# smdesai/mlx-swift-audio

Measured on AMD Instinct MI355X. Metric: audio-sec/s (Whisper large-v3-turbo b=32) at 1/2/4/8 GPU; codec samples/s, higher is better.
Workload: dtype bf16; 1 GPU; Whisper large-v3-turbo bf16, batch=32x30 s synthetic clips per MI355X, log-mel+encode+greedy decode (T=0, timestamps, max_tokens 448, one window per clip), random-init N(0,0.02^2) weights; clips_per_gpu=32, global_batch=32, parallelism=dp1, replicas=3, exchange=none, schedule=pipelined

## Files before the change

include/mia.h:

```cpp
#ifndef MIA_H
#define MIA_H

#include <stddef.h>
#include <stdint.h>

#ifdef __cplusplus
extern "C" {
#endif

typedef struct mia_ctx mia_ctx;
typedef struct mia_whisper mia_whisper;
typedef struct mia_codec mia_codec;
typedef struct mia_lm mia_lm;
typedef struct mia_s3tok mia_s3tok;

typedef enum {
  MIA_OK = 0,
  MIA_ERR_INVALID_ARGUMENT = -1,
  MIA_ERR_MODEL_NOT_LOADED = -2,
  MIA_ERR_INVALID_AUDIO = -3,
  MIA_ERR_OUT_OF_MEMORY = -4,
  MIA_ERR_DEVICE = -5,
  MIA_ERR_UNSUPPORTED = -6
} mia_status;
// ... 32 lines not shown

int mia_dp_shard_range(int n_items, int rank, int world, int* lo, int* hi);
int mia_dp_shard_cap(int n_items, int world);
int mia_dp_unpack_host(const int32_t* gathered, int n_items, int world, int L, int32_t* dense);
int mia_dp_available(void);
int mia_dp_unique_id(mia_ctx* ctx, void* id128);
int mia_dp_init(mia_ctx* ctx, int rank, int world, const void* unique_id);
int mia_dp_shutdown(mia_ctx* ctx);
int mia_dp_gather_tokens(mia_ctx* ctx, const int32_t* local_tokens, const int32_t* local_counts, int b_local, int L, int n_items,
                         int32_t* all_tokens, int32_t* all_counts);

int mia_op_linear(mia_ctx* ctx, const void* x, int64_t lda, const void* w, const float* bias, const float* r, int64_t ldr,
                  void* y, int64_t ldy, int M, int N, int K, int act, int dtype, int out_f32, int variant, int mem);

int mia_op_linear_epi(mia_ctx* ctx, const void* x, int64_t lda, const void* w, const float* bias, void* y, int64_t ldy, void* vt, int M, int N,
                      int K, int epi, int T, int H, int Tpad, int batch, int dtype, int out_f32, int variant, int mem);

int mia_op_attention_h64(mia_ctx* ctx, const void* qk, int64_t ld_qk, const void* vt, void* out, int64_t ld_out, int B, int T, int H, int Tpad,
                         int dtype, int mem);
int mia_op_attention_h64_variant(mia_ctx* ctx, const void* qk, int64_t ld_qk, const void* vt, void* out, int64_t ld_out, int B, int T, int H,
                                 int Tpad, int dtype, int variant, int mem);

int mia_op_conv1d_f32(mia_ctx* ctx, const float* x, int64_t ldx, int T_in, const float* w, const float* bias, const float* r, float* y,
                      int64_t ldy, int T_out, int N, int Cin, int taps, int stride, int dil, int pad, int act);

int mia_dequant_affine(mia_ctx* ctx, const uint32_t* wq, const void* scales, const void* biases, int64_t rows, int64_t cols,
                       int group_size, int bits, int scale_dtype, void* out, int out_dtype, int mem);

int mia_op_attention_f32(mia_ctx* ctx, const float* q, int64_t ldq, const float* k, int64_t ldk, const float* v, int64_t ldv, float* out,
                         int64_t ldo, int B, int T, int H, float scale);

typedef struct {
  const float* X; int64_t ldx; int32_t T_in;
  const float* W; int64_t ldw; int64_t w_phase_stride;
  const float* bias;
  const float* alpha; const float* ralpha;
  float lrelu_slope;
  float* Y; int64_t ldy; int32_t T_out;
  int32_t y_row_mul, y_row_off, y_phase_step;
  const float* R; const float* R2; int64_t ldr;
  const float* noise;
  float out_scale;
  int32_t M, N, Cin, taps, dil, pad;
  int32_t x_row_mul;
  int32_t act;
  int32_t tanh_out;
  const int32_t* phase_len; int32_t x_phase_step;
  int32_t n_seq; int64_t x_seq_step, y_seq_step;
  const int32_t* seq_len; const int32_t* noise_seq_off;
} mia_conv_gemm_desc;
int mia_op_conv_gemm_f32(mia_ctx* ctx, const mia_conv_gemm_desc* d, int phases);

int mia_op_attention_f32_ex(mia_ctx* ctx, const float* q, int64_t ldq, const float* k, int64_t ldk, const float* v, int64_t ldv, const float* p,
                            int64_t ldp, const float* bias_u, const float* bias_v, float* out, int64_t ldo, int B, int T, int H, float scale,
                            const int32_t* seq_len, int chunk);

int mia_op_attention_h128(mia_ctx* ctx, const void* q, int64_t ldq, const void* k, int64_t ldk, const void* v, int64_t ldv, void* out,
                          int64_t ldo, int B, int T, int H, float scale, const int32_t* seq_len, int dtype, int mem);

int mia_op_fsmn_add(mia_ctx* ctx, float* x, int64_t ldx, const void* v, int64_t ldv, const float* w, int B, int T, int D, int K, int left,
                    const int32_t* seq_len, int dtype, int mem);

int mia_op_funasr_logmel(mia_ctx* ctx, const float* pcm, const int64_t* offs, int B, float* mel_out, int mem);

int mia_op_kvq_attention(mia_ctx* ctx, const void* q, const void* k, const void* v, float* out, int Hq, int Hkv, int T, int dh, int bits,
                         int dtype);

int mia_op_lm_prompt_attention(mia_ctx* ctx, const void* q, const void* k, const void* v, float* out, int Hq, int Hkv, int T, int n, int dh,
                               int dtype);

typedef struct {
  const void* A; int64_t lda;
  const void* W;
  const uint32_t* wfrag; const float* stfrag; int32_t bits;
  int32_t w_frag;
  const float* bias;
  void* out; int64_t ldo;
  int32_t M, N, K, S, mode, dtype;
  float* xres; const float* nw; float* ss_out;
  const float* ss_in; int32_t ss_tiles, ss_dim; float eps, rs_scale;
  int32_t M_cap;
} mia_skinny_desc;
int mia_op_skinny_gemm(mia_ctx* ctx, const mia_skinny_desc* d);

typedef struct {
  int32_t n_mels, n_audio_ctx, n_audio_state, n_audio_head, n_audio_layer;
  int32_t n_vocab, n_text_ctx, n_text_state, n_text_head, n_text_layer;
} mia_whisper_dims;

typedef struct {
  const char* name;
  int32_t dtype;
  int32_t ndim;
  int64_t shape[4];
  const void* data;
} mia_tensor_view;

typedef struct {
  const int32_t* initial_tokens;
  int32_t n_initial;
  int32_t per_clip_initial;
  int32_t sot_index;
  const int32_t* suppress_ids;
  int32_t n_suppress;
  const int32_t* blank_ids;
  int32_t n_blank;
  int32_t eot, no_speech, no_timestamps, timestamp_begin;
  int32_t timestamps;
  int32_t max_tokens;
  int32_t max_initial_timestamp_index;
  int32_t max_new_tokens;
  float temperature;
  const float* uniforms;
  const int32_t* n_initial_per_clip;
  const int32_t* sot_index_per_clip;
  const float* clip_temperature;
  const int32_t* clip_active;
} mia_decode_opts;

mia_whisper* mia_whisper_load(mia_ctx* ctx, const mia_whisper_dims* dims, const mia_tensor_view* tensors, int n_tensors,
                              int compute_dtype);
void mia_whisper_free(mia_whisper* w);
mia_whisper* mia_whisper_clone(mia_whisper* src, mia_ctx* ctx);
int mia_whisper_attach_quantized(mia_whisper* w, const mia_tensor_view* tensors, int n_tensors, int group_size, int bits);
int mia_whisper_use_packed(mia_whisper* w, int on);
int mia_quant_repack(const uint32_t* codes, const void* scales, const void* biases, int N, int K, int bits, int scale_dtype,
                     int compute_dtype, uint32_t* wfrag, float* stfrag);
int mia_whisper_set_gemm_variant(mia_whisper* w, int variant);

int mia_whisper_set_debug(mia_whisper* w, int flags);
int mia_whisper_trace_logits(mia_whisper* w, const int32_t* clips, int n_clips);
int mia_whisper_read_logit_trace(mia_whisper* w, int slot, int first_pos, int n_pos, float* out);

int mia_whisper_encode(mia_whisper* w, const void* mel, int B, int mem);
int mia_whisper_get_audio_features(mia_whisper* w, void* out, int dtype, int mem);

int mia_whisper_decode_greedy(mia_whisper* w, const mia_decode_opts* opts, int32_t* tokens, int32_t* n_tokens,
                              float* avg_logprob, float* no_speech_prob, int mem);

int mia_whisper_detect_language(mia_whisper* w, int32_t sot, int32_t n_languages, int32_t* lang_idx, float* prob);

int mia_whisper_encode_windows(mia_whisper* w, const float* pcm, const int64_t* offs, int B, int64_t pad_right, int mem);
int mia_whisper_set_encode_stream(mia_whisper* w, void* hip_stream);
int mia_whisper_set_weight_sharing(mia_whisper* w, int concurrent_readers);
int mia_whisper_transcribe_windows(mia_whisper* w, const float* pcm, const int64_t* offs, int B, int64_t pad_right,
                                   const mia_decode_opts* opts, int32_t* tokens, int32_t* n_tokens, float* avg_logprob,
                                   float* no_speech_prob, int mem);

typedef struct mia_whisper_audio mia_whisper_audio;
mia_whisper_audio* mia_whisper_audio_create(mia_whisper* w, const float* pcm, const int64_t* offs, int n_clips, int64_t pad_right,
                                            int mem);
void mia_whisper_audio_free(mia_whisper_audio* a);
int64_t mia_whisper_audio_frames(const mia_whisper_audio* a);
int mia_whisper_audio_read(mia_whisper_audio* a, int clip, int64_t first_frame, int64_t n_frames, float* out);
int mia_whisper_encode_audio_windows(mia_whisper* w, mia_whisper_audio* a, const int32_t* clip, const int64_t* seek,
                                     const int32_t* n_valid, int B);

int mia_whisper_align(mia_whisper* w, const int32_t* tokens, int stride, const int32_t* n_tokens, const int32_t* heads, int n_heads,
                      const int32_t* num_frames, int row_start, int eot, float* token_probs, int32_t* text_idx, int32_t* time_idx,
                      int32_t* path_len, int path_cap, float* matrix);

typedef struct {
  int32_t latent_dim, decoder_dim;
  int32_t n_rates; int32_t decoder_rates[8];
  int32_t n_vq; int32_t vq_strides[4];
  int32_t codebook_size, codebook_dim;
// ... 188 lines not shown
```

mlx-swift-audio_amd/_abi.py:

```python
from __future__ import annotations

import ctypes as C

vp, cs, i32, i64, f32, f64, P = C.c_void_p, C.c_char_p, C.c_int, C.c_int64, C.c_float, C.c_double, C.POINTER


class ConvGemmDesc(C.Structure):
    _fields_ = [("X", vp), ("ldx", i64), ("T_in", i32),
                ("W", vp), ("ldw", i64), ("w_phase_stride", i64),
                ("bias", vp), ("alpha", vp), ("ralpha", vp), ("lrelu_slope", f32),
                ("Y", vp), ("ldy", i64), ("T_out", i32),
                ("y_row_mul", i32), ("y_row_off", i32), ("y_phase_step", i32),
                ("R", vp), ("R2", vp), ("ldr", i64), ("noise", vp), ("out_scale", f32),
                ("M", i32), ("N", i32), ("Cin", i32), ("taps", i32), ("dil", i32), ("pad", i32),
                ("x_row_mul", i32), ("act", i32), ("tanh_out", i32),
                ("phase_len", vp), ("x_phase_step", i32),
                ("n_seq", i32), ("x_seq_step", i64), ("y_seq_step", i64),
                ("seq_len", vp), ("noise_seq_off", vp)]


class SkinnyDesc(C.Structure):
    _fields_ = [("A", vp), ("lda", i64), ("W", vp),
                ("wfrag", vp), ("stfrag", vp), ("bits", i32), ("w_frag", i32),
                ("bias", vp), ("out", vp), ("ldo", i64),
# ... 101 lines not shown
    _fields_ = [("n_mels", i32), ("n_audio_state", i32), ("n_audio_head", i32), ("n_audio_layer", i32)]


class HiftConfig(C.Structure):
    _fields_ = [("in_channels", i32), ("base_channels", i32), ("nb_harmonics", i32), ("sampling_rate", i32),
                ("n_ups", i32), ("up_rates", i32 * 4), ("up_kernels", i32 * 4),
                ("n_res_kernels", i32), ("res_kernels", i32 * 4), ("src_res_kernels", i32 * 4),
                ("n_dilations", i32), ("dilations", i32 * 4),
                ("nsf_alpha", f32), ("nsf_sigma", f32), ("voiced_threshold", f32), ("lrelu_slope", f32), ("audio_limit", f32)]


class FlowConfig(C.Structure):
    _fields_ = [("input_size", i32), ("output_size", i32), ("spk_embed_dim", i32), ("vocab_size", i32),
                ("pre_lookahead_len", i32), ("n_timesteps", i32),
                ("enc_heads", i32), ("enc_linear_units", i32), ("enc_blocks", i32), ("enc_up_blocks", i32), ("upsample_stride", i32),
                ("dec_in_channels", i32), ("dec_channels", i32), ("dec_heads", i32), ("dec_n_blocks", i32), ("dec_mid_blocks", i32),
                ("cfg_rate", f32)]


STRUCTS = {
    "mia_conv_gemm_desc": ConvGemmDesc,
    "mia_skinny_desc": SkinnyDesc,
    "mia_whisper_dims": WhisperDims,
    "mia_tensor_view": TensorView,
    "mia_decode_opts": DecodeOpts,
    "mia_snac_config": SnacConfig,
    "mia_dac_config": DacConfig,
    "mia_dac_encoder_config": DacEncoderConfig,
    "mia_lm_config": LmConfig,
    "mia_lm_sampler": LmSampler,
    "mia_ras_params": RasParams,
    "mia_sensevoice_config": SensevoiceConfig,
    "mia_s3_config": S3Config,
    "mia_hift_config": HiftConfig,
    "mia_flow_config": FlowConfig,
}

TV = P(TensorView)

PROTOTYPES = {
    "mia_version": (cs, []),
    "mia_create": (vp, [i32]),
    "mia_create_on_stream": (vp, [i32, vp]),
    "mia_destroy": (None, [vp]),
    "mia_last_error": (cs, [vp]),
    "mia_stream": (vp, [vp]),
    "mia_synchronize": (i32, [vp]),
    "mia_profile_enable": (i32, [vp, i32]),
    "mia_profile_reset": (i32, [vp]),
    "mia_profile_read": (i32, [vp, cs, vp, vp, vp]),
    "mia_profile_codec_bytes": (f64, [i32]),
    "mia_logmel_whisper": (i32, [vp, vp, vp, i32, i32, i64, i64, vp, i32, i32]),
    "mia_logmel_s3": (i32, [vp, vp, vp, i32, i32, i64, i64, vp, i32, i32]),
    "mia_mel_s3gen_frames": (i64, [i64]),
    "mia_mel_s3gen": (i32, [vp, vp, i64, vp, i32]),
    "mia_resample_linear_len": (i64, [i64, f32]),
    "mia_resample_linear": (i32, [vp, vp, i64, f32, vp, i32]),
    "mia_resample_sinc_len": (i64, [i64, i32, i32]),
    "mia_resample_sinc_table": (i32, [i32, i32, vp, i32, vp, vp]),
    "mia_resample_sinc": (i32, [vp, vp, i64, i32, i32, vp, i64, vp, i32]),
    "mia_dp_shard_range": (i32, [i32, i32, i32, vp, vp]),
    "mia_dp_shard_cap": (i32, [i32, i32]),
    "mia_dp_unpack_host": (i32, [vp, i32, i32, i32, vp]),
    "mia_dp_available": (i32, []),
    "mia_dp_unique_id": (i32, [vp, vp]),
    "mia_dp_init": (i32, [vp, i32, i32, vp]),
    "mia_dp_shutdown": (i32, [vp]),
    "mia_dp_gather_tokens": (i32, [vp, vp, vp, i32, i32, i32, vp, vp]),
    "mia_op_linear": (i32, [vp, vp, i64, vp, vp, vp, i64, vp, i64] + [i32] * 8),
    "mia_op_linear_epi": (i32, [vp, vp, i64, vp, vp, vp, i64, vp] + [i32] * 12),
    "mia_op_attention_h64": (i32, [vp, vp, i64, vp, vp, i64] + [i32] * 6),
    "mia_op_attention_h64_variant": (i32, [vp, vp, i64, vp, vp, i64] + [i32] * 7),
    "mia_op_conv1d_f32": (i32, [vp, vp, i64, i32, vp, vp, vp, vp, i64] + [i32] * 8),
    "mia_dequant_affine": (i32, [vp, vp, vp, vp, i64, i64, i32, i32, i32, vp, i32, i32]),
    "mia_op_attention_f32": (i32, [vp, vp, i64, vp, i64, vp, i64, vp, i64, i32, i32, i32, f32]),
    "mia_op_conv_gemm_f32": (i32, [vp, P(ConvGemmDesc), i32]),
    "mia_op_attention_f32_ex": (i32, [vp, vp, i64, vp, i64, vp, i64, vp, i64, vp, vp, vp, i64, i32, i32, i32, f32, vp, i32]),
    "mia_op_attention_h128": (i32, [vp, vp, i64, vp, i64, vp, i64, vp, i64, i32, i32, i32, f32, vp, i32, i32]),
    "mia_op_fsmn_add": (i32, [vp, vp, i64, vp, i64, vp, i32, i32, i32, i32, i32, vp, i32, i32]),
    "mia_op_funasr_logmel": (i32, [vp, vp, vp, i32, vp, i32]),
    "mia_op_kvq_attention": (i32, [vp, vp, vp, vp, vp] + [i32] * 6),
    "mia_op_lm_prompt_attention": (i32, [vp, vp, vp, vp, vp] + [i32] * 6),
    "mia_op_skinny_gemm": (i32, [vp, P(SkinnyDesc)]),
    "mia_whisper_load": (vp, [vp, P(WhisperDims), TV, i32, i32]),
    "mia_whisper_free": (None, [vp]),
    "mia_whisper_clone": (vp, [vp, vp]),
    "mia_whisper_attach_quantized": (i32, [vp, TV, i32, i32, i32]),
    "mia_whisper_use_packed": (i32, [vp, i32]),
    "mia_quant_repack": (i32, [vp, vp, vp, i32, i32, i32, i32, i32, vp, vp]),
    "mia_whisper_set_gemm_variant": (i32, [vp, i32]),
    "mia_whisper_set_debug": (i32, [vp, i32]),
    "mia_whisper_trace_logits": (i32, [vp, vp, i32]),
    "mia_whisper_read_logit_trace": (i32, [vp, i32, i32, i32, vp]),
    "mia_whisper_encode": (i32, [vp, vp, i32, i32]),
    "mia_whisper_get_audio_features": (i32, [vp, vp, i32, i32]),
    "mia_whisper_decode_greedy": (i32, [vp, P(DecodeOpts), vp, vp, vp, vp, i32]),
    "mia_whisper_detect_language": (i32, [vp, i32, i32, vp, vp]),
    "mia_whisper_encode_windows": (i32, [vp, vp, vp, i32, i64, i32]),
    "mia_whisper_set_encode_stream": (i32, [vp, vp]),
    "mia_whisper_set_weight_sharing": (i32, [vp, i32]),
    "mia_whisper_transcribe_windows": (i32, [vp, vp, vp, i32, i64, P(DecodeOpts), vp, vp, vp, vp, i32]),
    "mia_whisper_audio_create": (vp, [vp, vp, vp, i32, i64, i32]),
    "mia_whisper_audio_free": (None, [vp]),
    "mia_whisper_audio_frames": (i64, [vp]),
    "mia_whisper_audio_read": (i32, [vp, i32, i64, i64, vp]),
    "mia_whisper_encode_audio_windows": (i32, [vp, vp, vp, vp, vp, i32]),
    "mia_whisper_align": (i32, [vp, vp, i32, vp, vp, i32, vp, i32, i32, vp, vp, vp, vp, i32, vp]),
    "mia_snac_load": (vp, [vp, P(SnacConfig), TV, i32]),
    "mia_dac_load": (vp, [vp, P(DacConfig), TV, i32]),
    "mia_codec_free": (None, [vp]),
    "mia_codec_output_len": (i64, [vp, i64]),
    "mia_codec_noise_len": (i64, [vp, i64]),
    "mia_snac_decode": (i32, [vp, vp, vp, i32, vp, i64, vp, i64, vp, i32]),
    "mia_dac_decode": (i32, [vp, vp, i32, i64, vp, i64, vp, i32]),
    "mia_snac_decode_batch": (i32, [vp, i32, vp, vp, i32, vp, i64, vp, vp, vp, i32]),
    "mia_dac_decode_batch": (i32, [vp, i32, vp, i32, vp, vp, vp, vp, i32]),
    "mia_codec_set_stack_budget": (i32, [vp, i64]),
    "mia_dac_load_encoder": (i32, [vp, P(DacEncoderConfig), TV, i32]),
    "mia_dac_code_len": (i64, [vp, i64]),
    "mia_dac_encode": (i32, [vp, vp, i64, i32, vp, i64, vp, i32]),
    "mia_mimi_load": (vp, [vp, vp, TV, i32]),
    "mia_mimi_free": (None, [vp]),
    "mia_mimi_output_len": (i64, [vp, i64]),
    "mia_mimi_decode": (i32, [vp, vp, i32, i64, vp, i64, vp, i32]),
    "mia_mimi_stream_create": (vp, [vp]),
    "mia_mimi_stream_free": (None, [vp]),
    "mia_mimi_stream_reset": (i32, [vp]),
    "mia_mimi_stream_decode": (i32, [vp, vp, i32, i64, vp, i64, vp, i32]),
    "mia_speaker_audio_create": (vp, [vp, vp, i64, i32, f32, f32]),
    "mia_speaker_audio_free": (None, [vp]),
    "mia_speaker_audio_len": (i64, [vp]),
    "mia_speaker_audio_data": (vp, [vp]),
    "mia_speaker_audio_read": (i32, [vp, i64, i64, vp]),
    "mia_speaker_audio_features": (i32, [vp, vp, vp, i32, vp, vp]),
    "mia_speaker_audio_launches": (i32, [vp]),
    "mia_op_rfft_block": (i64, []),
    "mia_op_rfft_pow2": (i32, [vp, vp, i64, i64, vp]),
    "mia_clip_create": (vp, [vp, vp, i64, i32]),
    "mia_clip_free": (None, [vp]),
    "mia_clip_len": (i64, [vp]),
    "mia_clip_data": (vp, [vp]),
    "mia_clip_read": (i32, [vp, i64, i64, vp]),
    "mia_clip_speech_bounds": (i32, [vp, i64, i64, f32, vp, vp, vp]),
    "mia_clip_frame_energy": (i32, [vp, i64, i64, i64, i64, vp]),
    "mia_clip_num_frames": (i64, [i64, i64, i64]),
    "mia_clip_launches": (i32, [vp]),
    "mia_lm_load": (vp, [vp, P(LmConfig), TV, i32, i32]),
    "mia_lm_attach_quantized": (i32, [vp, TV, i32, i32, i32]),
    "mia_lm_attach_q4": (i32, [vp, TV, i32, i32]),
    "mia_lm_use_q4": (i32, [vp, i32]),
    "mia_lm_set_debug": (i32, [vp, i32]),
    "mia_lm_set_prompt_attention": (i32, [vp, i32]),
    "mia_lm_free": (None, [vp]),
    "mia_lm_reset": (i32, [vp]),
    "mia_lm_forward": (i32, [vp, vp, i32, vp]),
    "mia_lm_generate": (i32, [vp, vp, i32, P(LmSampler), vp, vp, vp]),
    "mia_lm_set_batch": (i32, [vp, i32]),
    "mia_lm_generate_batch": (i32, [vp, vp, vp, i32, P(LmSampler), vp, vp, vp]),
    "mia_lm_set_kv_quant": (i32, [vp, i32, i32]),
    "mia_lm_read_kv": (i32, [vp, i32, i32, i32, i32, vp, vp]),
    "mia_lm_generate_ras": (i32, [vp, vp, i32, P(RasParams), vp, i32, vp, vp]),
    "mia_lm_generate_ras_batch": (i32, [vp, vp, vp, i32, P(RasParams), vp, i32, vp, i32, vp]),
    "mia_lm_generate_greedy": (i32, [vp, vp, i32, vp, i32, i32, vp, vp]),
    "mia_lm_generate_greedy_batch": (i32, [vp, vp, vp, i32, vp, i32, i32, vp, i32, vp]),
    "mia_lm_generate_topk": (i32, [vp, vp, i32, f32, i32, f32, vp, i32, i32, vp, vp, vp]),
    "mia_lm_generate_topk_batch": (i32, [vp, vp, vp, i32, f32, i32, f32, vp, i32, i32, vp, vp, i32, vp]),
# ... 43 lines not shown
```

mlx-swift-audio_amd/csrc/decode.h:

```cpp
#pragma once
#include "skinny.h"
#include "whisper.h"

int dec_launch_embed_ln(mia_whisper* w, const LNW& ln, hipStream_t s);
int dec_launch_reduce_ln(mia_whisper* w, int S, const float* bias, const LNW& ln, hipStream_t s);
int dec_launch_skinny(mia_whisper* w, const SkinnyArgs& a, int mode, hipStream_t s);
int dec_launch_skinny_q(mia_whisper* w, const SkinnyArgs& a, const uint32_t* wfrag, const float* stfrag, int bits, int mode, hipStream_t s);
int dec_launch_lnfold(const void* w16, int N, int K, const float* gamma, const float* beta, float* c1, float* c2, int dtype, hipStream_t s, const float* bias = nullptr);
int dec_launch_attention(mia_whisper* w, const void* q, const void* kc, const void* vc, void* out, int fixed_keys, int cap_keys,
                         hipStream_t s, float* qk_out = nullptr, const int32_t* head_slot = nullptr, int n_slots = 0, int qk_ctx = 0,
                         bool self_nt = false);
bool dec_head_is_split(const DecodeParams& p);
int dec_launch_trace(mia_whisper* w, hipStream_t s);
int dec_launch_head(mia_whisper* w, int32_t* last_ts, const DecodeParams& p, hipStream_t s);
int dec_launch_finalize(mia_whisper* w, int32_t* out_n, const DecodeParams& p, hipStream_t s);
```

mlx-swift-audio_amd/csrc/decode_kernels.hip:

```cpp
#include <cstdlib>

#include <type_traits>
#include "decode.h"

constexpr int ROW_NV = 2;

__device__ __forceinline__ float block256_sum(float v, float* sh) {
  v = wave_sum(v);
  __syncthreads();
  if ((threadIdx.x & 63) == 0) sh[threadIdx.x >> 6] = v;
  __syncthreads();
  return (sh[0] + sh[1]) + (sh[2] + sh[3]);
}

template <typename T>
__device__ __forceinline__ void row_layernorm_store(const f32x4 (&v)[ROW_NV], int nv, int D, const float* __restrict__ gamma,
                                                    const float* __restrict__ beta, uint16_t* __restrict__ h, int row, float* sh) {
  const int tid = threadIdx.x;
  f32x4 gm[ROW_NV], bt[ROW_NV];
#pragma unroll
  for (int i = 0; i < ROW_NV; ++i) {
    const bool in = tid + 256 * i < nv;
    gm[i] = in ? *reinterpret_cast<const f32x4*>(gamma + 4 * (tid + 256 * i)) : (f32x4){0.f, 0.f, 0.f, 0.f};
    bt[i] = in ? *reinterpret_cast<const f32x4*>(beta + 4 * (tid + 256 * i)) : (f32x4){0.f, 0.f, 0.f, 0.f};
// ... 129 lines not shown
#pragma unroll
        for (int j = 0; j < 8; ++j) dot += qf[j] * T::to_f32((uint16_t)kv[u][j]);
        dot += dpp_xor1(dot);
        dot += dpp_xor2(dot);
        dot += dpp_half_mirror(dot);
        const int key = k0 + 8 * u + g;
        if (c == 0 && key < nk) sc[key] = dot * scale;
      }
      if (more) {
#pragma unroll
        for (int u = 0; u < U; ++u) kv[u] = kn[u];
      }
    }
  }
  s16x8 vv[U], vn[U];
  if (wave * (8 * U) < nk) load_trip(vv, rv, wave * (8 * U));
  __syncthreads();
  if (qk_out && head_slot[h] >= 0) {
    float* dst = qk_out + (((int64_t)b * n_slots + head_slot[h]) * qk_ctx + pos_arr[b]) * nk;
    for (int i = tid; i < nk; i += 256) dst[i] = sc[i];
  }
  float m = -INFINITY;
  for (int i = tid; i < nk; i += 256) m = fmaxf(m, sc[i]);
  m = wave_max(m);
  if (lane == 0) red2[wave] = m;
  __syncthreads();
  m = fmaxf(fmaxf(red2[0], red2[1]), fmaxf(red2[2], red2[3]));
  float sum = 0.f;
  for (int i = tid; i < nk; i += 256) { const float p = __expf(sc[i] - m); sc[i] = p; sum += p; }
  sum = wave_sum(sum);
  if (lane == 0) red2[4 + wave] = sum;
  __syncthreads();
  sum = (red2[4] + red2[5]) + (red2[6] + red2[7]);
  float acc[8];
#pragma unroll
  for (int j = 0; j < 8; ++j) acc[j] = 0.f;
  for (int k0 = wave * (8 * U); k0 < nk; k0 += TRIP) {
    const bool more = k0 + TRIP < nk;
    if (more) load_trip(vn, rv, k0 + TRIP);
    float pw[U];
#pragma unroll
    for (int u = 0; u < U; ++u) {
      const int key = k0 + 8 * u + g;
      pw[u] = key < nk ? sc[key] : 0.f;
    }
#pragma unroll
    for (int u = 0; u < U; ++u)
#pragma unroll
      for (int j = 0; j < 8; ++j) acc[j] += pw[u] * T::to_f32((uint16_t)vv[u][j]);
    if (more) {
#pragma unroll
      for (int u = 0; u < U; ++u) vv[u] = vn[u];
    }
  }
#pragma unroll
  for (int j = 0; j < 8; ++j) {
    acc[j] += dpp_xor8(acc[j]);
    acc[j] += __shfl_xor(acc[j], 16, 64);
    acc[j] += __shfl_xor(acc[j], 32, 64);
  }
  if (g == 0) {
#pragma unroll
    for (int j = 0; j < 8; ++j) red[wave][c * 8 + j] = acc[j];
  }
  __syncthreads();
  if (tid < 64) {
    const float o = ((red[0][tid] + red[1][tid]) + (red[2][tid] + red[3][tid])) / sum;
    out[afrag_index(b, h * 64 + tid, D)] = T::from_f32(o);
  }
}

struct HeadBufs {
  const float* logits;
  int32_t* tokens;
  int32_t* n_gen;
  int32_t* finished;
  int32_t* last_ts;
  float* sum_logprob;
  int32_t* n_logprob;
  float* no_speech;
  const uint32_t* suppress;
  const float* uniforms;
  DecClip clip;
};

constexpr int HEAD_NPT = 52;
struct ArgMax { float v; int i; };
__device__ __forceinline__ ArgMax amax(ArgMax a, ArgMax b) {
  return (b.v > a.v || (b.v == a.v && b.i < a.i)) ? b : a;
}
__device__ __forceinline__ ArgMax wave_amax(ArgMax a) {
#define AMAX_STEP(CTRL) { const ArgMax b{dpp_f32<CTRL>(a.v), dpp_i32<CTRL>(a.i)}; a = amax(a, b); }
  AMAX_STEP(0xB1) AMAX_STEP(0x4E) AMAX_STEP(0x141) AMAX_STEP(0x140)
#undef AMAX_STEP
  ArgMax r = ArgMax{lane_f32(a.v, 0), __builtin_amdgcn_readlane(a.i, 0)};
  r = amax(r, ArgMax{lane_f32(a.v, 16), __builtin_amdgcn_readlane(a.i, 16)});
  r = amax(r, ArgMax{lane_f32(a.v, 32), __builtin_amdgcn_readlane(a.i, 32)});
  r = amax(r, ArgMax{lane_f32(a.v, 48), __builtin_amdgcn_readlane(a.i, 48)});
  return r;
}

struct HeadRule {
  bool active;
  bool decide;
  bool heuristic, sup_ts_all, sup_text_below_eot, sup_below_tsb;
  int ts_floor;
  int max_first;
  int num_gen, cur_len;
};
__device__ __forceinline__ HeadRule head_rule(const HeadBufs& hb, const DecodeParams& p, int b) {
  HeadRule r{};
  const int pos = hb.clip.pos[b], n_initial = hb.clip.n_init[b], sot_index = hb.clip.sot_idx[b];
  r.cur_len = pos + 1;
  const bool generating = r.cur_len >= n_initial;
  r.active = !(generating && hb.finished[b]) && (generating || pos == sot_index);
  r.decide = generating;
  r.num_gen = r.cur_len - n_initial;
  r.max_first = p.V;
  if (r.active && r.decide && p.timestamps) {
    const int32_t* toks = hb.tokens + (int64_t)b * p.n_ctx;
    const int tsb = p.timestamp_begin;
    const int last = toks[r.cur_len - 1];
    const bool last_was_ts = r.num_gen >= 1 && last >= tsb;
    const bool penult_was_ts = r.num_gen < 2 || toks[r.cur_len - 2] >= tsb;
    if (last_was_ts) { if (penult_was_ts) r.sup_ts_all = true; else r.sup_text_below_eot = true; }
    const int lt = hb.last_ts[b];
    if (lt > 0) r.ts_floor = penult_was_ts ? lt + 1 : lt;
    if (r.num_gen == 0) {
      r.sup_below_tsb = true;
      const int last_allowed = tsb + p.max_initial_ts;
      if (last_allowed < p.V) r.max_first = last_allowed;
    }
    r.heuristic = r.num_gen > 0;
  }
  return r;
}

__device__ __forceinline__ bool head_masked(const HeadRule& r, const DecodeParams& p, const uint32_t* bits, int i) {
  const int tsb = p.timestamp_begin;
  if ((bits[i >> 5] >> (i & 31)) & 1u) return true;
  if (p.timestamps) {
    if (i == p.no_timestamps) return true;
    if (r.sup_ts_all && i >= tsb) return true;
    if (r.sup_text_below_eot && i < p.eot) return true;
    if (i >= tsb && i < r.ts_floor) return true;
    if (r.sup_below_tsb && i < tsb) return true;
    if (i > r.max_first) return true;
  }
  return false;
}

struct HeadPart { float mx_text, mx_ts, s_all, s_ts, bAv, bBv, fA, fB; int bAi, bBi; };
constexpr int HEAD_NONE = 0x7fffffff;
template <int NPT> using HeadKept = std::conditional_t<(NPT > 32), unsigned long long, unsigned>;

template <int NTH, int NPT>
__device__ __forceinline__ void head_load(float (&x)[NPT], const float* lg, int base, int V) {
#pragma unroll
  for (int u = 0; u < NPT; ++u) { const int i = base + (int)threadIdx.x + NTH * u; x[u] = i < V ? lg[i] : -INFINITY; }
}

template <int NTH, int NPT>
__device__ __forceinline__ HeadPart head_reduce(const float (&x)[NPT], int base, const HeadRule& r, const HeadBufs& hb, const DecodeParams& p,
                                                HeadKept<NPT>& okA) {
  constexpr int NWV = NTH / 64;
  __shared__ float shf[NWV][4];
  __shared__ float sha[NWV][2];
  __shared__ int shai[NWV][2];
  const int tid = threadIdx.x, lane = tid & 63, wave = tid >> 6;
  const int V = p.V, tsb = p.timestamp_begin;
  const uint32_t* bits = hb.suppress + (r.num_gen == 0 ? (V + 31) / 32 : 0);
  float mx_text = -INFINITY, mx_ts = -INFINITY;
  ArgMax bA{-INFINITY, HEAD_NONE}, bB{-INFINITY, HEAD_NONE};
  okA = 0;
#pragma unroll
  for (int u = 0; u < NPT; ++u) {
    const int i = base + tid + NTH * u;
    if (i >= V) continue;
    if (i >= tsb) mx_ts = fmaxf(mx_ts, x[u]); else mx_text = fmaxf(mx_text, x[u]);
    if (r.decide && !head_masked(r, p, bits, i)) {
      okA |= (HeadKept<NPT>)1 << u;
      bA = amax(bA, ArgMax{x[u], i});
      if (i >= tsb) bB = amax(bB, ArgMax{x[u], i});
    }
  }
  mx_text = wave_max(mx_text); mx_ts = wave_max(mx_ts);
  bA = wave_amax(bA); bB = wave_amax(bB);
  if (lane == 0) { shf[wave][0] = mx_text; shf[wave][1] = mx_ts; sha[wave][0] = bA.v; shai[wave][0] = bA.i; sha[wave][1] = bB.v; shai[wave][1] = bB.i; }
  __syncthreads();
  mx_text = shf[0][0]; mx_ts = shf[0][1]; bA = ArgMax{sha[0][0], shai[0][0]}; bB = ArgMax{sha[0][1], shai[0][1]};
  for (int w2 = 1; w2 < NWV; ++w2) {
    mx_text = fmaxf(mx_text, shf[w2][0]); mx_ts = fmaxf(mx_ts, shf[w2][1]);
    bA = amax(bA, ArgMax{sha[w2][0], shai[w2][0]}); bB = amax(bB, ArgMax{sha[w2][1], shai[w2][1]});
  }
  const float mx_all = fmaxf(mx_text, mx_ts);
  __syncthreads();
  float s_all = 0.f, s_ts = 0.f, fA = 0.f, fB = 0.f;
#pragma unroll
  for (int u = 0; u < NPT; ++u) {
    const int i = base + tid + NTH * u;
    if (i >= V) continue;
    s_all += __expf(x[u] - mx_all);
    if (r.heuristic && i >= tsb) s_ts += __expf(x[u] - mx_ts);
    if ((okA >> u) & 1) {
      fA += __expf(x[u] - bA.v);
      if (r.heuristic && i >= tsb) fB += __expf(x[u] - bB.v);
    }
  }
  s_all = wave_sum(s_all); s_ts = wave_sum(s_ts); fA = wave_sum(fA); fB = wave_sum(fB);
  if (lane == 0) { shf[wave][0] = s_all; shf[wave][1] = s_ts; shf[wave][2] = fA; shf[wave][3] = fB; }
  __syncthreads();
  s_all = s_ts = fA = fB = 0.f;
  for (int w2 = 0; w2 < NWV; ++w2) { s_all += shf[w2][0]; s_ts += shf[w2][1]; fA += shf[w2][2]; fB += shf[w2][3]; }
  return HeadPart{mx_text, mx_ts, s_all, s_ts, bA.v, bB.v, fA, fB, bA.i, bB.i};
}

struct HeadPick { float lse; bool useB, all_masked; ArgMax best; float fsum; int next; };
__device__ __forceinline__ HeadPick head_decide(const HeadRule& r, const HeadPart& m) {
  HeadPick k;
  k.lse = fmaxf(m.mx_text, m.mx_ts) + __logf(m.s_all);
  k.useB = false;
  if (r.heuristic) {
    const float ts_lse = (m.mx_ts - k.lse) + __logf(m.s_ts);
    const float max_text = m.mx_text - k.lse;
    k.useB = ts_lse > max_text;
  }
  k.best = k.useB ? ArgMax{m.bBv, m.bBi} : ArgMax{m.bAv, m.bAi};
  k.fsum = k.useB ? m.fB : m.fA;
  k.all_masked = k.best.i == HEAD_NONE;
  k.next = k.all_masked ? 0 : k.best.i;
  return k;
}

__device__ __forceinline__ void head_probe(const HeadBufs& hb, const DecodeParams& p, int b, const HeadRule& r, float lse) {
  if (r.active && r.cur_len - 1 == hb.clip.sot_idx[b]) hb.no_speech[b] = __expf(hb.logits[(int64_t)b * p.V + p.no_speech] - lse);
}

__device__ __forceinline__ int head_commit(const HeadBufs& hb, const DecodeParams& p, int b, const HeadRule& r, const HeadPick& k, int next) {
  const int pos = r.cur_len - 1, n_initial = r.cur_len - r.num_gen;
  int newpos = -1;
  if (!r.decide) newpos = pos + 1;
  else if (r.active) {
    if (next != p.eot) {
      hb.sum_logprob[b] += k.all_masked ? __int_as_float(0x7fc00000) : (hb.logits[(int64_t)b * p.V + next] - k.best.v) - __logf(k.fsum);
      hb.n_logprob[b] += 1;
    }
    hb.tokens[(int64_t)b * p.n_ctx + r.cur_len] = next;
    hb.n_gen[b] = r.num_gen + 1;
    if (next > p.timestamp_begin) hb.last_ts[b] = next;
    int cap = p.max_tokens - n_initial;
    if (p.max_new_tokens > 0 && p.max_new_tokens < cap) cap = p.max_new_tokens;
    if (next == p.eot || r.num_gen + 1 >= cap) hb.finished[b] = 1;
    else newpos = pos + 1;
  }
  if (newpos >= 0) hb.clip.pos[b] = newpos;
  return newpos;
}

__global__ __launch_bounds__(1024) void dec_head(HeadBufs hb, DecodeParams p) {
  __shared__ float seg[HEAD_NPT * 16];
  __shared__ int s_pick[2];
  __shared__ float s_val[2];
  const int b = blockIdx.x, tid = threadIdx.x, lane = tid & 63, wave = tid >> 6;
  const HeadRule r = head_rule(hb, p, b);
  if (!r.active) {
    if (tid == 0) head_commit(hb, p, b, r, HeadPick{}, 0);
    return;
  }
  const int tsb = p.timestamp_begin;
  float x[HEAD_NPT];
  head_load<1024, HEAD_NPT>(x, hb.logits + (int64_t)b * p.V, 0, p.V);
  HeadKept<HEAD_NPT> okA;
  const HeadPart m = head_reduce<1024, HEAD_NPT>(x, 0, r, hb, p, okA);
  const HeadPick k = head_decide(r, m);
  if (tid == 0) head_probe(hb, p, b, r, k.lse);
  int next = k.next;
  const float temperature = hb.clip.temp[b];
  if (r.decide && temperature > 0.0f && !k.all_masked) {
    const float inv_t = 1.0f / temperature;
    auto weight = [&](int u) -> float {
      const int i = tid + 1024 * u;
      const bool kept = ((okA >> u) & 1ull) && (!k.useB || i >= tsb);
      return kept ? __expf((x[u] - k.best.v) * inv_t) : 0.f;
    };
#pragma unroll
    for (int u = 0; u < HEAD_NPT; ++u) {
      const float ssum = wave_sum(weight(u));
      if (lane == 0) seg[u * 16 + wave] = ssum;
    }
    __syncthreads();
    if (tid == 0) {
      float total = 0.f;
      for (int j = 0; j < HEAD_NPT * 16; ++j) total += seg[j];
      const float rnd = hb.uniforms[(int64_t)b * p.n_ctx + r.num_gen];
      const float goal = rnd * total;
      float cum = 0.f; int sel = -1;
      for (int j = 0; j < HEAD_NPT * 16; ++j) {
        if (seg[j] > 0.f && cum + seg[j] >= goal) { sel = j; break; }
        cum += seg[j];
      }
      if (sel < 0) { for (int j = HEAD_NPT * 16 - 1; j >= 0; --j) if (seg[j] > 0.f) { sel = j; break; } cum -= 0.f; }
      s_pick[0] = sel; s_val[0] = cum; s_val[1] = goal;
    }
    __syncthreads();
    const int sel = s_pick[0];
    if (sel >= 0 && wave == (sel & 15)) {
      const int u_sel = sel >> 4;
      float mine = 0.f;
#pragma unroll
      for (int u = 0; u < HEAD_NPT; ++u) if (u == u_sel) mine = weight(u);
      float incl = mine;
#pragma unroll
      for (int o = 1; o < 64; o <<= 1) { const float t = __shfl_up(incl, o, 64); if (lane >= o) incl += t; }
      const unsigned long long hit = __ballot(mine > 0.f && s_val[0] + incl >= s_val[1]);
      const unsigned long long any = __ballot(mine > 0.f);
      int ln = hit ? __ffsll((long long)hit) - 1 : 63 - __clzll((long long)any);
      if (lane == 0) s_pick[1] = 1024 * u_sel + 64 * wave + ln;
    }
    __syncthreads();
    if (sel >= 0) next = s_pick[1];
  }
  if (tid == 0) head_commit(hb, p, b, r, k, next);
}

constexpr int HEAD_SPLIT = 32;
constexpr int HEAD_NPT2 = 7;

__global__ __launch_bounds__(256) void dec_head_partial(HeadBufs hb, DecodeParams p, HeadPart* __restrict__ parts) {
  const int k = blockIdx.x, b = blockIdx.y;
  const int base = k * (256 * HEAD_NPT2);
  float x[HEAD_NPT2];
  head_load<256, HEAD_NPT2>(x, hb.logits + (int64_t)b * p.V, base, p.V);
  const HeadRule r = head_rule(hb, p, b);
  if (!r.active) return;
  HeadKept<HEAD_NPT2> okA;
  const HeadPart part = head_reduce<256, HEAD_NPT2>(x, base, r, hb, p, okA);
  if (threadIdx.x == 0) parts[b * HEAD_SPLIT + k] = part;
}

struct NextEmbed { const uint16_t* emb; const float* pos_emb; const float* gamma; const float* beta; float* x; uint16_t* h; int D; };

template <typename T>
__global__ __launch_bounds__(256) void dec_head_final(HeadBufs hb, DecodeParams p, const HeadPart* __restrict__ parts, NextEmbed ne) {
  __shared__ int s_newpos;
  __shared__ float sh[4];
  const int b = blockIdx.x, tid = threadIdx.x;
  float mx_text = -INFINITY, mx_ts = -INFINITY, s_all = 0.f, s_ts = 0.f, fA = 0.f, fB = 0.f;
  ArgMax bA{-INFINITY, HEAD_NONE}, bB{-INFINITY, HEAD_NONE};
  const HeadRule r = head_rule(hb, p, b);
  if (tid < 64 && r.active) {
    HeadPart me{-INFINITY, -INFINITY, 0.f, 0.f, -INFINITY, -INFINITY, 0.f, 0.f, HEAD_NONE, HEAD_NONE};
    if (tid < HEAD_SPLIT) me = parts[b * HEAD_SPLIT + tid];
    mx_text = wave_max(me.mx_text); mx_ts = wave_max(me.mx_ts);
    bA = wave_amax(ArgMax{me.bAv, me.bAi}); bB = wave_amax(ArgMax{me.bBv, me.bBi});
    const float mx_all = fmaxf(mx_text, mx_ts);
    const float ml = fmaxf(me.mx_text, me.mx_ts);
    s_all = wave_sum(ml > -INFINITY ? me.s_all * __expf(ml - mx_all) : 0.f);
    s_ts = wave_sum(me.mx_ts > -INFINITY ? me.s_ts * __expf(me.mx_ts - mx_ts) : 0.f);
    fA = wave_sum(me.bAv > -INFINITY ? me.fA * __expf(me.bAv - bA.v) : 0.f);
    fB = wave_sum(me.bBv > -INFINITY ? me.fB * __expf(me.bBv - bB.v) : 0.f);
  }
  if (tid == 0) {
    const HeadPick k = head_decide(r, HeadPart{mx_text, mx_ts, s_all, s_ts, bA.v, bB.v, fA, fB, bA.i, bB.i});
    head_probe(hb, p, b, r, k.lse);
    s_newpos = head_commit(hb, p, b, r, k, k.next);
  }
  __syncthreads();
  const int np_ = s_newpos;
  if (np_ < 0 || np_ >= p.n_ctx) return;
  const int D = ne.D, nv = D >> 2;
  const int tok = hb.tokens[(int64_t)b * p.n_ctx + np_];
  const uint16_t* e = ne.emb + (int64_t)tok * D;
  const float* pe = ne.pos_emb + (int64_t)np_ * D;
  float* xr = ne.x + (int64_t)b * D;
  f32x4 v[ROW_NV];
#pragma unroll
  for (int i = 0; i < ROW_NV; ++i) {
    const int c = tid + 256 * i;
    if (c < nv) {
      const s16x4 ev = *reinterpret_cast<const s16x4*>(e + 4 * c);
      const f32x4 pv = *reinterpret_cast<const f32x4*>(pe + 4 * c);
#pragma unroll
      for (int j = 0; j < 4; ++j) v[i][j] = T::to_f32((uint16_t)ev[j]) + pv[j];
      *reinterpret_cast<f32x4*>(xr + 4 * c) = v[i];
    } else v[i] = (f32x4){0.f, 0.f, 0.f, 0.f};
  }
  row_layernorm_store<T>(v, nv, D, ne.gamma, ne.beta, ne.h, b, sh);
}

__global__ void dec_finalize(const int32_t* __restrict__ tokens, const int32_t* __restrict__ n_gen,
                             const float* __restrict__ sum_lp, const int32_t* __restrict__ n_lp, int32_t* __restrict__ out_tokens,
                             int32_t* __restrict__ out_n, float* __restrict__ out_avg, const int32_t* __restrict__ n_init, DecodeParams p) {
  const int b = blockIdx.x;
  const int32_t* t = tokens + (int64_t)b * p.n_ctx + n_init[b];
  __shared__ int n_keep;
  if (threadIdx.x == 0) {
    int n = n_gen[b];
    for (int i = 0; i < n; ++i) if (t[i] == p.eot) { n = i; break; }
    n_keep = n;
    out_n[b] = n;
    out_avg[b] = n_lp[b] > 0 ? sum_lp[b] / (float)n_lp[b] : 0.0f;
  }
  __syncthreads();
  for (int i = threadIdx.x; i < p.max_tokens; i += blockDim.x) out_tokens[(int64_t)b * p.max_tokens + i] = i < n_keep ? t[i] : 0;
}

int dec_launch_embed_ln(mia_whisper* w, const LNW& ln, hipStream_t s) {
  const int D = w->dims.n_text_state;
  if (w->dtype == MIA_F16)
    hipLaunchKernelGGL(dec_embed_ln<F16>, dim3(w->cur_B), dim3(256), 0, s, w->tokens, (const uint16_t*)w->tok_emb, w->dec_pos, ln.g, ln.b, w->dx, (uint16_t*)w->dh, w->clip.pos, D, w->dims.n_text_ctx);
  else
    hipLaunchKernelGGL(dec_embed_ln<BF16>, dim3(w->cur_B), dim3(256), 0, s, w->tokens, (const uint16_t*)w->tok_emb, w->dec_pos, ln.g, ln.b, w->dx, (uint16_t*)w->dh, w->clip.pos, D, w->dims.n_text_ctx);
  return 0;
}

int dec_launch_reduce_ln(mia_whisper* w, int S, const float* bias, const LNW& ln, hipStream_t s) {
  const int D = w->dims.n_text_state;
  if (w->dtype == MIA_F16)
    hipLaunchKernelGGL(dec_reduce_ln<F16>, dim3(w->cur_B), dim3(256), 0, s, w->partial, S, w->cur_B, bias, ln.g, ln.b, w->dx, (uint16_t*)w->dh, D);
  else
    hipLaunchKernelGGL(dec_reduce_ln<BF16>, dim3(w->cur_B), dim3(256), 0, s, w->partial, S, w->cur_B, bias, ln.g, ln.b, w->dx, (uint16_t*)w->dh, D);
  return 0;
}

int dec_launch_attention(mia_whisper* w, const void* q, const void* kc, const void* vc, void* out, int fixed_keys, int cap_keys,
                         hipStream_t s, float* qk_out, const int32_t* head_slot, int n_slots, int qk_ctx, bool self_nt) {
  if (cap_keys > DEC_MAX_KEYS) return -1;
  dim3 grid(w->dims.n_text_head, w->cur_B), block(256);
#define ATT(T_, U_, NTL_)                                                                                                            \
  hipLaunchKernelGGL((dec_attention<T_, U_, NTL_>), grid, block, 0, s, (const uint16_t*)q, (const uint16_t*)kc, (const uint16_t*)vc,   \
                     (uint16_t*)out, w->clip.pos, fixed_keys, cap_keys, w->dims.n_text_head, 0.125f, qk_out, head_slot, n_slots, qk_ctx)
  const bool nt = fixed_keys > 0 || self_nt;
  if (w->dtype == MIA_F16) { if (nt) ATT(F16, 4, true); else ATT(F16, 4, false); }
  else { if (nt) ATT(BF16, 4, true); else ATT(BF16, 4, false); }
#undef ATT
  return 0;
}

bool dec_head_is_split(const DecodeParams& p) {
  return p.greedy && !p.head_single && p.V <= 256 * HEAD_NPT2 * HEAD_SPLIT;
}

__global__ __launch_bounds__(256) void dec_trace_logits(const float* __restrict__ logits, const int32_t* __restrict__ pos, const int32_t* __restrict__ clips,
                                                        float* __restrict__ trace, int V, int n_ctx) {
  const int slot = blockIdx.y, b = clips[slot];
  const int p = pos[b];
  if (p < 0 || p >= n_ctx) return;
  const float* src = logits + (int64_t)b * V;
  float* dst = trace + ((int64_t)slot * n_ctx + p) * V;
  for (int i = blockIdx.x * 256 + threadIdx.x; i < V; i += gridDim.x * 256) dst[i] = src[i];
}

int dec_launch_trace(mia_whisper* w, hipStream_t s) {
  if (!w->trace || w->trace_n <= 0) return -1;
  hipLaunchKernelGGL(dec_trace_logits, dim3(32, w->trace_n), dim3(256), 0, s, w->logits, w->clip.pos, w->trace_clips, w->trace, w->dims.n_vocab, w->dims.n_text_ctx);
  return 0;
}

int dec_launch_head(mia_whisper* w, int32_t* last_ts, const DecodeParams& p, hipStream_t s) {
  if (p.V > 1024 * HEAD_NPT) return -1;
  HeadBufs hb{w->logits, w->tokens, w->n_gen, w->finished, last_ts, w->sum_logprob, w->n_logprob, w->no_speech, w->suppress_bits, w->uniforms, w->clip};
  if (dec_head_is_split(p)) {
    HeadPart* parts = reinterpret_cast<HeadPart*>(w->partial);
    hipLaunchKernelGGL(dec_head_partial, dim3(HEAD_SPLIT, w->cur_B), dim3(256), 0, s, hb, p, parts);
    const LNW& ln0 = w->dec[0].attn_ln;
    NextEmbed ne{(const uint16_t*)w->tok_emb, w->dec_pos, ln0.g, ln0.b, w->dx, (uint16_t*)w->dh, w->dims.n_text_state};
    if (w->dtype == MIA_F16) hipLaunchKernelGGL(dec_head_final<F16>, dim3(w->cur_B), dim3(256), 0, s, hb, p, (const HeadPart*)parts, ne);
    else hipLaunchKernelGGL(dec_head_final<BF16>, dim3(w->cur_B), dim3(256), 0, s, hb, p, (const HeadPart*)parts, ne);
    return 0;
  }
  hipLaunchKernelGGL(dec_head, dim3(w->cur_B), dim3(1024), 0, s, hb, p);
  return 0;
}

int dec_launch_finalize(mia_whisper* w, int32_t* out_n, const DecodeParams& p, hipStream_t s) {
  hipLaunchKernelGGL(dec_finalize, dim3(w->cur_B), dim3(256), 0, s, w->tokens, w->n_gen, w->sum_logprob, w->n_logprob, w->out_tokens, out_n, w->out_avg, w->clip.n_init, p);
  return 0;
}
```

mlx-swift-audio_amd/csrc/ops_abi.hip:

```cpp
#include "gemm.h"
#include "mia_internal.h"
#include "ops.h"

extern "C" int mia_op_linear(mia_ctx* ctx, const void* x, int64_t lda, const void* w, const float* bias, const float* r, int64_t ldr,
                             void* y, int64_t ldy, int M, int N, int K, int act, int dtype, int out_f32, int variant, int mem) {
  if (!ctx) return MIA_ERR_INVALID_ARGUMENT;
  MIA_CHECK_ARG(ctx, x && w && y, "op_linear: null pointer");
  MIA_CHECK_ARG(ctx, dtype == MIA_BF16 || dtype == MIA_F16, "op_linear: dtype must be MIA_BF16 or MIA_F16");
  MIA_CHECK_ARG(ctx, HostIo::valid(mem), "op_linear: bad mem");
  MIA_CHECK_ARG(ctx, M > 0 && N > 0 && K > 0 && lda >= K && ldy >= N && (!r || ldr >= N), "op_linear: bad shape");
  MIA_HIP(ctx, hipSetDevice(ctx->device));
  HostIo io(ctx, mem);
  GemmArgs g;
  g.M = M; g.N = N; g.K = K; g.lda = lda; g.ldc = ldy; g.ldr = ldr; g.act = act; g.out_f32 = out_f32 ? 1 : 0; g.variant = variant;
  const size_t xb = (size_t)M * lda * 2, wb = (size_t)N * K * 2, yb = (size_t)M * ldy * (out_f32 ? 4 : 2);
  const size_t bb = bias ? (size_t)N * 4 : 0, rb = r ? (size_t)M * ldr * 4 : 0;
  Carve cv;
  const size_t o_x = cv.add(io.staged(xb)), o_w = cv.add(io.staged(wb)), o_y = cv.add(io.staged(yb)), o_b = cv.add(io.staged(bb)), o_r = cv.add(io.staged(rb));
  char* ws;
  if (!cv.workspace(ctx, ws)) return MIA_ERR_OUT_OF_MEMORY;
  g.A = io.in(x, ws + o_x, xb); g.W = io.in(w, ws + o_w, wb); g.bias = io.in(bias, ws + o_b, bb); g.R = io.in(r, ws + o_r, rb);
  g.C = io.out(y, ws + o_y, yb);
  if (const char* e = mia_gemm_check(g)) return mia_fail(ctx, MIA_ERR_INVALID_ARGUMENT, "%s", e);
  if (mia_gemm_launch(g, dtype, ctx->stream) != 0) return mia_fail(ctx, MIA_ERR_DEVICE, "op_linear: launch failed");
// ... 80 lines not shown
static const char* conv_gemm_abi_check(const ConvGemmArgs& g, int phases) {
  if (!g.X || !g.W || !g.Y) return "null pointer";
  if (phases <= 0 || g.T_in <= 0 || g.T_out <= 0 || g.dil <= 0 || g.x_row_mul <= 0) return "bad argument";
  if (g.ldx < g.Cin || g.ldy < g.N || ((g.R || g.R2) && g.ldr < g.N)) return "row strides must cover the row";
  if (g.gelu < 0 || g.gelu > 6) return "unknown activation";
  return nullptr;
}

extern "C" int mia_op_conv1d_f32(mia_ctx* ctx, const float* x, int64_t ldx, int T_in, const float* w, const float* bias, const float* r, float* y,
                                 int64_t ldy, int T_out, int N, int Cin, int taps, int stride, int dil, int pad, int act) {
  if (!ctx) return MIA_ERR_INVALID_ARGUMENT;
  MIA_CHECK_ARG(ctx, x && w && y && T_in > 0 && T_out > 0 && N > 0 && taps > 0 && stride > 0 && dil > 0, "op_conv1d_f32: bad argument");
  MIA_HIP(ctx, hipSetDevice(ctx->device));
  ConvGemmArgs g;
  g.X = x; g.ldx = ldx; g.T_in = T_in; g.W = w; g.bias = bias; g.Y = y; g.ldy = ldy; g.T_out = T_out; g.R = r; g.ldr = ldy;
  g.M = T_out; g.N = N; g.Cin = Cin; g.taps = taps; g.dil = dil; g.pad = pad; g.x_row_mul = stride; g.gelu = act;
  if (const char* e = conv_gemm_abi_check(g, 1)) return mia_fail(ctx, MIA_ERR_INVALID_ARGUMENT, "op_conv1d_f32: %s", e);
  if (const char* e = codec_conv_gemm_check(g)) return mia_fail(ctx, MIA_ERR_INVALID_ARGUMENT, "%s", e);
  if (codec_conv_gemm_launch(g, 1, ctx->stream)) return mia_fail(ctx, MIA_ERR_DEVICE, "op_conv1d_f32: launch failed");
  return MIA_OK;
}

extern "C" int mia_op_conv_gemm_f32(mia_ctx* ctx, const mia_conv_gemm_desc* d, int phases) {
  if (!ctx) return MIA_ERR_INVALID_ARGUMENT;
  MIA_CHECK_ARG(ctx, d, "op_conv_gemm_f32: null descriptor");
  MIA_HIP(ctx, hipSetDevice(ctx->device));
  ConvGemmArgs g;
  g.X = d->X; g.ldx = d->ldx; g.T_in = d->T_in; g.W = d->W; g.ldw = d->ldw; g.w_phase_stride = d->w_phase_stride; g.bias = d->bias;
  g.alpha = d->alpha; g.ralpha = d->ralpha; g.lrelu_slope = d->lrelu_slope; g.Y = d->Y; g.ldy = d->ldy; g.T_out = d->T_out;
  g.y_row_mul = d->y_row_mul; g.y_row_off = d->y_row_off; g.y_phase_step = d->y_phase_step; g.R = d->R; g.R2 = d->R2; g.ldr = d->ldr;
  g.noise = d->noise; g.out_scale = d->out_scale; g.M = d->M; g.N = d->N; g.Cin = d->Cin; g.taps = d->taps; g.dil = d->dil; g.pad = d->pad;
  g.x_row_mul = d->x_row_mul; g.gelu = d->act; g.tanh_out = d->tanh_out; g.phase_len = d->phase_len; g.x_phase_step = d->x_phase_step;
  g.n_seq = d->n_seq; g.x_seq_step = d->x_seq_step; g.y_seq_step = d->y_seq_step; g.seq_len = d->seq_len; g.noise_seq_off = d->noise_seq_off;
  if (const char* e = conv_gemm_abi_check(g, phases)) return mia_fail(ctx, MIA_ERR_INVALID_ARGUMENT, "op_conv_gemm_f32: %s", e);
  return codec_conv_gemm_run(ctx, g, phases, "op_conv_gemm_f32");
}

#include "skinny.h"
static const char* skinny_abi_check(const mia_skinny_desc& d) {
  if (d.dtype != MIA_BF16 && d.dtype != MIA_F16) return "dtype must be MIA_BF16 or MIA_F16";
  if (d.mode != SK_OUTF32 && d.mode != SK_PARTIAL && d.mode != SK_SWIGLU && d.mode != SK_RESID) return "mode must be 1 (OUTF32), 2 (PARTIAL), 4 (SWIGLU) or 5 (RESID)";
  if (!d.A || !d.out) return "null pointer";
  if (d.wfrag ? !d.stfrag : !d.W) return "null weights";
  if (d.lda < d.K) return "lda must cover the row";
  if (d.mode != SK_PARTIAL && d.S != 1) return "only PARTIAL takes S > 1";
  if ((d.mode == SK_OUTF32 || d.mode == SK_RESID) && d.ldo < d.N) return "ldo must cover the row";
  if (d.mode == SK_SWIGLU && d.ldo < d.N / 2) return "ldo must cover the row";
  if (d.mode == SK_RESID && (!d.xres || !d.nw || !d.ss_out)) return "RESID needs xres, nw and ss_out";
  if (d.M_cap < 0) return "bad M_cap";
  auto misaligned = [](const void* p) { return ((uintptr_t)p & 15) != 0; };
  if (misaligned(d.A) || misaligned(d.W) || misaligned(d.wfrag) || misaligned(d.stfrag) || misaligned(d.out) || misaligned(d.xres) || misaligned(d.nw) ||
      (d.mode == SK_RESID && misaligned(d.bias)))
    return "operands must be 16-byte aligned";
  return nullptr;
}

extern "C" int mia_op_skinny_gemm(mia_ctx* ctx, const mia_skinny_desc* d) {
  if (!ctx) return MIA_ERR_INVALID_ARGUMENT;
  MIA_CHECK_ARG(ctx, d, "op_skinny_gemm: null descriptor");
  if (const char* e = skinny_abi_check(*d)) return mia_fail(ctx, MIA_ERR_INVALID_ARGUMENT, "op_skinny_gemm: %s", e);
  MIA_HIP(ctx, hipSetDevice(ctx->device));
  SkinnyArgs a{(const uint16_t*)d->A, d->lda, (const uint16_t*)d->W, d->bias, d->out, d->ldo, nullptr, nullptr, nullptr, d->M, d->N, d->K, d->S, MIA_ACT_NONE, 0, 0, 0};
  a.xres = d->xres; a.nw = d->nw; a.ss_out = d->ss_out;
  a.ss_in = d->ss_in; a.ss_tiles = d->ss_tiles; a.ss_dim = d->ss_dim; a.eps = d->eps; a.rs_scale = d->rs_scale;
  int rc;
  if (d->wfrag) rc = skinny_gemm_q_launch(a, d->wfrag, d->stfrag, d->bits, d->mode, d->dtype, ctx->stream, d->M_cap);
  else {
    if (d->w_frag) {
      MIA_CHECK_ARG(ctx, d->N > 0 && d->K > 0 && d->K % 32 == 0 && ((uint64_t)d->N + 15) / 16 * 16 * (uint64_t)d->K * 2 <= 0xffffffffull,
                    "op_skinny_gemm: N, K must be positive, K a multiple of 32, W below 4 GiB");
      void* wf = mia_workspace(ctx, (size_t)((d->N + 15) / 16) * 16 * d->K * 2);
      if (!wf) return MIA_ERR_OUT_OF_MEMORY;
      if (dec_launch_repack_wfrag(d->W, wf, d->N, d->K, ctx->stream)) return mia_fail(ctx, MIA_ERR_DEVICE, "op_skinny_gemm: fragment repack failed");
      a.W = (const uint16_t*)wf; a.w_frag = 1;
    }
    rc = skinny_gemm_launch(a, d->mode, d->dtype, ctx->stream);
  }
  if (rc) return mia_fail(ctx, MIA_ERR_INVALID_ARGUMENT, "op_skinny_gemm: the launcher refused the arguments (K %d, S %d, lda %lld, N %d, ldo %lld, mode %d, bits %d, ss_tiles %d)",
                          d->K, d->S, (long long)d->lda, d->N, (long long)d->ldo, d->mode, d->bits, d->ss_tiles);
  if (hipGetLastError() != hipSuccess) return mia_fail(ctx, MIA_ERR_DEVICE, "op_skinny_gemm: launch failed");
  return MIA_OK;
}

extern "C" int mia_op_attention_f32_ex(mia_ctx* ctx, const float* q, int64_t ldq, const float* k, int64_t ldk, const float* v, int64_t ldv,
                                       const float* p, int64_t ldp, const float* bias_u, const float* bias_v, float* out, int64_t ldo, int B, int T,
                                       int H, float scale, const int32_t* seq_len, int chunk) {
  if (!ctx) return MIA_ERR_INVALID_ARGUMENT;
  MIA_CHECK_ARG(ctx, chunk >= 0 && (int64_t)B * T < (1ll << 31), "op_attention_f32: bad argument");
  MIA_HIP(ctx, hipSetDevice(ctx->device));
  AttnF32Args a;
  a.q = q; a.ldq = ldq; a.k = k; a.ldk = ldk; a.v = v; a.ldv = ldv; a.out = out; a.ldo = ldo; a.B = B; a.T = T; a.H = H; a.scale = scale;
  a.p = p; a.ldp = ldp; a.bias_u = bias_u; a.bias_v = bias_v; a.seq_len = seq_len; a.chunk = chunk;
  if (const char* e = mia_attn_f32_check(a)) return mia_fail(ctx, MIA_ERR_INVALID_ARGUMENT, "%s", e);
  if (mia_attn_f32_launch(a, ctx->stream)) return mia_fail(ctx, MIA_ERR_DEVICE, "op_attention_f32: launch failed");
  return MIA_OK;
}
extern "C" int mia_op_attention_f32(mia_ctx* ctx, const float* q, int64_t ldq, const float* k, int64_t ldk, const float* v, int64_t ldv, float* out,
                                    int64_t ldo, int B, int T, int H, float scale) {
  return mia_op_attention_f32_ex(ctx, q, ldq, k, ldk, v, ldv, nullptr, 0, nullptr, nullptr, out, ldo, B, T, H, scale, nullptr, 0);
}

extern "C" int mia_op_attention_h128(mia_ctx* ctx, const void* q, int64_t ldq, const void* k, int64_t ldk, const void* v, int64_t ldv, void* out,
                                     int64_t ldo, int B, int T, int H, float scale, const int32_t* seq_len, int dtype, int mem) {
  if (!ctx) return MIA_ERR_INVALID_ARGUMENT;
  MIA_CHECK_ARG(ctx, HostIo::valid(mem), "op_attention_h128: bad mem");
  MIA_CHECK_ARG(ctx, q && k && v && out && B > 0 && T > 0 && H > 0 && (int64_t)B * T < (1ll << 31), "op_attention_h128: bad argument");
  MIA_HIP(ctx, hipSetDevice(ctx->device));
  Attn128Args a;
  a.ldq = ldq; a.ldk = ldk; a.ldv = ldv; a.ldo = ldo; a.B = B; a.T = T; a.H = H; a.scale = scale; a.dtype = dtype;
  const int64_t rows = (int64_t)B * T, D = (int64_t)H * 128;
  HostIo io(ctx, mem);
  MIA_CHECK_ARG(ctx, !io.host() || (ldq >= D && ldk >= D && ldv >= D && ldo >= D), "op_attention_h128: row strides must be >= H * 128");
  const size_t qb = (size_t)((rows - 1) * ldq + D) * 2, kb = (size_t)((rows - 1) * ldk + D) * 2, vb = (size_t)((rows - 1) * ldv + D) * 2;
  const size_t ob = (size_t)((rows - 1) * ldo + D) * 2, sb = (size_t)B * 4;
  Carve cv;
  const size_t o_q = cv.add(io.staged(qb)), o_k = cv.add(io.staged(kb)), o_v = cv.add(io.staged(vb)), o_o = cv.add(io.staged(ob)), o_s = cv.add(io.staged(sb));
  char* ws;
  if (!cv.workspace(ctx, ws)) return MIA_ERR_OUT_OF_MEMORY;
  a.q = io.in(q, ws + o_q, qb); a.k = io.in(k, ws + o_k, kb); a.v = io.in(v, ws + o_v, vb);
  a.out = io.inout(out, ws + o_o, ob);
  a.seq_len = io.in(seq_len, ws + o_s, sb);
  if (const char* e = mia_attn128_check(a)) return mia_fail(ctx, MIA_ERR_INVALID_ARGUMENT, "%s", e);
  if (mia_attn128_launch(a, ctx->stream)) return mia_fail(ctx, MIA_ERR_DEVICE, "op_attention_h128: launch failed");
  return io.finish();
}

extern "C" int mia_op_fsmn_add(mia_ctx* ctx, float* x, int64_t ldx, const void* v, int64_t ldv, const float* w, int B, int T, int D, int K, int left,
                               const int32_t* seq_len, int dtype, int mem) {
  if (!ctx) return MIA_ERR_INVALID_ARGUMENT;
  MIA_CHECK_ARG(ctx, HostIo::valid(mem), "op_fsmn_add: bad mem");
  MIA_CHECK_ARG(ctx, x && v && w && B > 0 && T > 0 && D > 0 && K > 0 && (int64_t)B * T < (1ll << 31), "op_fsmn_add: bad argument");
  MIA_HIP(ctx, hipSetDevice(ctx->device));
  FsmnArgs a;
  a.ldx = ldx; a.ldv = ldv; a.B = B; a.T = T; a.D = D; a.K = K; a.left = left; a.dtype = dtype;
  const int64_t rows = (int64_t)B * T;
  HostIo io(ctx, mem);
  MIA_CHECK_ARG(ctx, !io.host() || (ldx >= D && ldv >= D), "op_fsmn_add: row strides must be >= D");
  const size_t xb = (size_t)((rows - 1) * ldx + D) * 4, vb = (size_t)((rows - 1) * ldv + D) * 2, wb = (size_t)K * D * 4, sb = (size_t)B * 4;
  Carve cv;
  const size_t o_x = cv.add(io.staged(xb)), o_v = cv.add(io.staged(vb)), o_w = cv.add(io.staged(wb)), o_s = cv.add(io.staged(sb));
  char* ws;
  if (!cv.workspace(ctx, ws)) return MIA_ERR_OUT_OF_MEMORY;
  a.x = io.inout(x, ws + o_x, xb);
  a.v = io.in(v, ws + o_v, vb); a.w = io.in(w, ws + o_w, wb); a.seq_len = io.in(seq_len, ws + o_s, sb);
  if (const char* e = mia_fsmn_check(a)) return mia_fail(ctx, MIA_ERR_INVALID_ARGUMENT, "%s", e);
  if (mia_fsmn_launch(a, ctx->stream)) return mia_fail(ctx, MIA_ERR_DEVICE, "op_fsmn_add: launch failed");
  return io.finish();
}

#include "lm.h"
namespace {

float widen16(uint16_t x, int dtype) {
  if (dtype == MIA_F16) { _Float16 h; memcpy(&h, &x, 2); return (float)h; }
  const uint32_t u = (uint32_t)x << 16; float f; memcpy(&f, &u, 4); return f;
}

struct LmOpRows {
  std::vector<float> part;
  std::vector<int2> rowmap;
  int Nq = 0, N = 0;
  float* d_part = nullptr; int2* d_map = nullptr; uint16_t* d_q = nullptr; uint16_t* d_att = nullptr; char* extra = nullptr;
  mia_lm sh;

  void build(const void* q, const void* k, const void* v, int Hq, int Hkv, int T, int n, int dh, int dtype) {
    const int Nk = Hkv * dh;
// ... 91 lines not shown
```

mlx-swift-audio_amd/csrc/skinny.h:

```cpp
#pragma once
#include <cmath>
#include <hip/hip_runtime.h>
#include <stdint.h>

#include "../../include/mia.h"
#include "tensor_loader.h"

enum { SK_OUT16 = 0, SK_OUTF32 = 1, SK_PARTIAL = 2, SK_QKV = 3, SK_SWIGLU = 4, SK_RESID = 5 };

__host__ __device__ inline int64_t afrag_index(int m, int k, int K) {
  return ((((int64_t)(m >> 5) * (K >> 5) + (k >> 5)) * 2 + ((m >> 4) & 1)) * 64 + ((k >> 3) & 3) * 16 + (m & 15)) * 8 + (k & 7);
}
__host__ __device__ inline int64_t wfrag_index(int n, int k, int K) {
  return (((int64_t)(n >> 4) * (K >> 5) + (k >> 5)) * 64 + ((k >> 3) & 3) * 16 + (n & 15)) * 8 + (k & 7);
}

struct SkinnyArgs {
  const uint16_t* A; int64_t lda;
  const uint16_t* W;
  const float* bias;
  void* out; int64_t ldo;
  uint16_t* cache_k; uint16_t* cache_v;
  const int32_t* pos;
  int M, N, K, S, act, D, H, n_ctx;
  int out_frag = 0;
  int w_frag = 0;
  int w_keep = 0;
  float* xres = nullptr; const float* nw = nullptr; float* ss_out = nullptr;
  const float* ss_in = nullptr; int ss_tiles = 0; int ss_dim = 0; float eps = 0.f;
  float rs_scale = 1.f;
  const float* c1 = nullptr; const float* c2 = nullptr;
};

inline float mia_carry_prescale(const float* gain, int n, int dtype) {
  if (dtype != MIA_F16) return 1.f;
  float mx = 0.f;
  for (int i = 0; i < n; ++i) { const float a = fabsf(gain[i]); if (a > mx) mx = a; }
  if (!(mx > 0.f) || !std::isfinite(mx)) return 1.f;
  int k = 3 + ilogbf(mx);
  k = k < -24 ? -24 : (k > 40 ? 40 : k);
  return ldexpf(1.f, -k);
}

inline float* mia_carry_gain(TensorLoader& L, const std::vector<float>& g, int dtype, float* plain, float* rs) {
  const float p = mia_carry_prescale(g.data(), (int)g.size(), dtype);
  *rs = 1.f / p;
  if (p == 1.f) return plain;
  std::vector<float> v(g);
  for (float& x : v) x *= p;
  return L.up(v);
}

int dec_launch_repack_wfrag(const void* src, void* dst, int N, int K, hipStream_t s);
bool dec_wfrag_copy(const void* src, int N, int K, std::vector<void*>& allocs, hipStream_t s, void** dst);
int skinny_gemm_launch(const SkinnyArgs& a, int mode, int dtype, hipStream_t s);
int skinny_gemm_q_launch(const SkinnyArgs& a, const uint32_t* wfrag, const float* stfrag, int bits, int mode, int dtype, hipStream_t s, int M_cap = 0);
```

mlx-swift-audio_amd/csrc/skinny_frag.hip:

```cpp
#include "decode.h"
#include "skinny_device.h"

template <typename T>
__global__ __launch_bounds__(256) void repack_wfrag(const uint16_t* __restrict__ src, uint16_t* __restrict__ dst, int N, int K) {
  const int64_t chunk = (int64_t)blockIdx.x * 256 + threadIdx.x;
  const int ksteps = K >> 5;
  const int64_t total = (int64_t)((N + 15) >> 4) * ksteps * 64;
  if (chunk >= total) return;
  const int lane = (int)(chunk & 63);
  const int64_t tk = chunk >> 6;
  const int kstep = (int)(tk % ksteps), tile = (int)(tk / ksteps);
  const int n = tile * 16 + (lane & 15), k = kstep * 32 + 8 * (lane >> 4);
  s16x8 v = (s16x8){0, 0, 0, 0, 0, 0, 0, 0};
  if (n < N) v = *reinterpret_cast<const s16x8*>(src + (int64_t)n * K + k);
  *reinterpret_cast<s16x8*>(dst + chunk * 8) = v;
}

int dec_launch_repack_wfrag(const void* src, void* dst, int N, int K, hipStream_t s) {
  if (N <= 0 || K <= 0 || K % 32 != 0) return -1;
  const int64_t total = (int64_t)((N + 15) / 16) * (K / 32) * 64;
  hipLaunchKernelGGL(repack_wfrag<BF16>, dim3((unsigned)((total + 255) / 256)), dim3(256), 0, s, (const uint16_t*)src, (uint16_t*)dst, N, K);
  return hipGetLastError() == hipSuccess ? 0 : -1;
}

// ... 174 lines not shown
  lnstat.issue(a, z * 32, wave, lane);
  const int ksteps = a.K >> 5, tiles = (a.N + 15) >> 4;
  const int per_wave = ksteps / (a.S * NW);
  const int ks0 = (split * NW + wave) * per_wave;
  const uint16_t* wp[NT];
#pragma unroll
  for (int t = 0; t < NT; ++t) {
    int tile = blockIdx.x * NT + t; tile = tile < tiles ? tile : tiles - 1;
    wp[t] = a.W + (((int64_t)tile * ksteps + ks0) * 64 + lane) * 8;
  }
  const uint16_t* ap = a.A + ((((int64_t)z * ksteps + ks0) * 2) * 64 + lane) * 8;
  const SkinnyPre<NT> pre = skinny_prefetch<MODE, NT>(a, blockIdx.x * (16 * NT), z * 32, lane);
  f32x4 acc[NT][2];
#pragma unroll
  for (int t = 0; t < NT; ++t) { acc[t][0] = (f32x4){0.f, 0.f, 0.f, 0.f}; acc[t][1] = (f32x4){0.f, 0.f, 0.f, 0.f}; }
  struct Batch { s16x8 w[KB][NT], a0[KB], a1[KB]; };
  const bool keep = a.w_keep != 0;
  const WFragBuf wb(a);
  const WFragBuf ab(a, 0);
  const uint32_t ao = ab.offset(ap);
  uint32_t wo[NT];
#pragma unroll
  for (int t = 0; t < NT; ++t) wo[t] = wb.offset(wp[t]);
  auto load_batch = [&](Batch& t, int ks) {
    auto go = [&](auto keep_tag) {
      constexpr int AUX = decltype(keep_tag)::value ? 0 : 2;
#pragma unroll
      for (int u = 0; u < KB; ++u) {
#pragma unroll
        for (int n = 0; n < NT; ++n) t.w[u][n] = wb.template load<AUX>(wo[n] + 1024u * (uint32_t)(ks + u));
        t.a0[u] = ab.template load<0>(ao + 2048u * (uint32_t)(ks + u));
        t.a1[u] = ab.template load<0>(ao + 2048u * (uint32_t)(ks + u) + 1024u);
      }
    };
    if (keep) go(std::true_type{}); else go(std::false_type{});
  };
  auto mma_batch = [&](const Batch& t) {
#pragma unroll
    for (int u = 0; u < KB; ++u)
#pragma unroll
      for (int n = 0; n < NT; ++n) {
        acc[n][0] = T::mfma16(t.w[u][n], t.a0[u], acc[n][0]);
        acc[n][1] = T::mfma16(t.w[u][n], t.a1[u], acc[n][1]);
      }
  };
  const int nb = per_wave / KB;
  int ks = 0;
  if (nb > 0) {
    Batch b0, b1, b2, b3;
    load_batch(b0, 0);
    if (nb > 1) load_batch(b1, KB);
    if (nb > 2) load_batch(b2, 2 * KB);
    lnstat.finish(a, st, lane);
    for (int i = 0; i < nb; i += 4) {
      if (i + 3 < nb) load_batch(b3, (i + 3) * KB);
      mma_batch(b0);
      if (i + 1 >= nb) break;
      if (i + 4 < nb) load_batch(b0, (i + 4) * KB);
      mma_batch(b1);
      if (i + 2 >= nb) break;
      if (i + 5 < nb) load_batch(b1, (i + 5) * KB);
      mma_batch(b2);
      if (i + 3 >= nb) break;
      if (i + 6 < nb) load_batch(b2, (i + 6) * KB);
      mma_batch(b3);
    }
    ks = nb * KB;
  } else lnstat.finish(a, st, lane);
  for (; ks < per_wave; ++ks) {
    const s16x8 fa0 = *reinterpret_cast<const s16x8*>(ap + 1024 * ks);
    const s16x8 fa1 = *reinterpret_cast<const s16x8*>(ap + 1024 * ks + 512);
#pragma unroll
    for (int n = 0; n < NT; ++n) {
      const s16x8 fw = *reinterpret_cast<const s16x8*>(wp[n] + 512 * ks);
      acc[n][0] = T::mfma16(fw, fa0, acc[n][0]);
      acc[n][1] = T::mfma16(fw, fa1, acc[n][1]);
    }
  }
  if (!skinny_wave_reduce<NT, NW>(acc, wave, lane)) return;
  if constexpr (MODE == SK_RESID) skinny_resid_frag<T, NT>(a, acc, blockIdx.x * (16 * NT), z * 32, lane);
  else skinny_epilogue_v<T, MODE, NT>(a, acc, pre, blockIdx.x * (16 * NT), z * 32, split, lane, st);
}

template <typename T, int MODE>
static int skinny_frag_launch_m(const SkinnyArgs& a, hipStream_t s) {
  const int tiles = (a.N + 15) / 16, zb = (a.M + 31) / 32, ksteps = a.K / 32;
  if constexpr (MODE == SK_OUTF32) {
    hipLaunchKernelGGL((dec_skinny_fring<T, MODE, 4, 2, 1>), dim3((tiles + 3) / 4, a.S, zb), dim3(64), 0, s, a);
    return 0;
  } else {
    const int per_split = ksteps / a.S;
    const dim3 grid(tiles, a.S, zb);
    if constexpr (MODE == SK_RESID) {
      if (per_split == 160) { hipLaunchKernelGGL((dec_skinny_fring<T, MODE, 1, 2, 16>), grid, dim3(1024), 0, s, a); return 0; }
      if (per_split == 80) { hipLaunchKernelGGL((dec_skinny_fflat<T, MODE, 1, 10, 8>), grid, dim3(512), 0, s, a); return 0; }
      if (per_split == 40) { hipLaunchKernelGGL((dec_skinny_fflat<T, MODE, 1, 5, 8>), grid, dim3(512), 0, s, a); return 0; }
      if (per_split % 16 == 0 && per_split >= 64) { hipLaunchKernelGGL((dec_skinny_fring<T, MODE, 1, 1, 16>), grid, dim3(1024), 0, s, a); return 0; }
      if (per_split % 8 == 0 && per_split >= 16) { hipLaunchKernelGGL((dec_skinny_fring<T, MODE, 1, 1, 8>), grid, dim3(512), 0, s, a); return 0; }
    }
    const int NW = per_split % 4 == 0 ? 4 : per_split % 2 == 0 ? 2 : 1;
    const int nstep = per_split / NW;
#define FF(NS_)                                                                                                       \
    if (NW == 4 && nstep == NS_) { hipLaunchKernelGGL((dec_skinny_fflat<T, MODE, 1, NS_, 4>), grid, dim3(256), 0, s, a); return 0; }
    FF(10) FF(5) FF(8) FF(6) FF(4) FF(3) FF(2) FF(1)
#undef FF
    if (NW == 4) hipLaunchKernelGGL((dec_skinny_fring<T, MODE, 1, 1, 4>), grid, dim3(256), 0, s, a);
    else if (NW == 2) hipLaunchKernelGGL((dec_skinny_fring<T, MODE, 1, 1, 2>), grid, dim3(128), 0, s, a);
    else hipLaunchKernelGGL((dec_skinny_fring<T, MODE, 1, 1, 1>), grid, dim3(64), 0, s, a);
    return 0;
  }
}

template <typename T>
static int skinny_frag_launch_t(const SkinnyArgs& a, int mode, hipStream_t s) {
  switch (mode) {
    case SK_OUT16: return skinny_frag_launch_m<T, SK_OUT16>(a, s);
    case SK_OUTF32: return skinny_frag_launch_m<T, SK_OUTF32>(a, s);
    case SK_PARTIAL: return skinny_frag_launch_m<T, SK_PARTIAL>(a, s);
    case SK_QKV: return skinny_frag_launch_m<T, SK_QKV>(a, s);
    case SK_RESID: return skinny_frag_launch_m<T, SK_RESID>(a, s);
    default: return -1;
  }
}

int dec_launch_skinny(mia_whisper* w, const SkinnyArgs& a, int mode, hipStream_t s) {
  if (!a.A || !a.W || !a.out || a.M <= 0 || a.N <= 0 || a.S <= 0 || a.K % (32 * a.S) != 0) return -1;
  if (mode == SK_QKV && (a.D % 64 != 0 || a.N != 3 * a.D || (a.ldo & 3) || !a.cache_k || !a.cache_v || !a.pos)) return -1;
  if (mode == SK_OUT16 && a.out_frag && a.N % 32 != 0) return -1;
  if (mode == SK_RESID && (a.S != 1 || a.N % 32 != 0 || !a.xres || !a.nw || !a.ss_out)) return -1;
  if (a.c1 && (!a.c2 || !a.ss_in || a.ss_tiles <= 0 || a.ss_tiles > 128 || a.ss_dim <= 0)) return -1;
  return w->dtype == MIA_F16 ? skinny_frag_launch_t<F16>(a, mode, s) : skinny_frag_launch_t<BF16>(a, mode, s);
}
```

mlx-swift-audio_amd/csrc/whisper.h:

```cpp
#pragma once
#include <map>
#include <string>
#include <vector>

#include "gemm.h"
#include "mia_device.h"
#include "mia_internal.h"
#include "ops.h"

struct LinearW {
  void* w = nullptr;
  void* wf = nullptr;
  float* b = nullptr;
  float* c1 = nullptr;
  float* c2 = nullptr;
  float ln_rs = 1.f;
  uint32_t* qw = nullptr;
  float* qst = nullptr;
  int N = 0, K = 0;
};

struct LNW {
  float* g = nullptr;
  float* b = nullptr;
  float* gc = nullptr;
};

struct EncBlockW {
  LNW attn_ln, mlp_ln;
  LinearW qkv, out, mlp1, mlp2;
};

struct DecBlockW {
  LNW attn_ln, cross_ln, mlp_ln;
  LinearW qkv, out;
  LinearW cq, ck, cv, cout;
  LinearW mlp1, mlp2;
};

struct DecClip {
  int32_t* pos;
  int32_t* n_init;
  int32_t* sot_idx;
  float* temp;
};

struct DecodeParams {
  int B, V, D, H, L, n_ctx;
  int eot, no_speech, no_timestamps, timestamp_begin;
  int timestamps, max_tokens, max_initial_ts, max_new_tokens;
  int greedy;
  int trace;
  int head_single;
  int split_ln;
  int packed;
  int keep_layers;
  int keep_vocab;
  int self_nt;
};

struct mia_whisper {
  mia_ctx* ctx = nullptr;
  mia_whisper_dims dims{};
  int dtype = MIA_BF16;
  int kpad_conv1 = 0;
  int gemm_variant = 3;
  std::vector<void*> allocs;
  std::vector<void*> batch_allocs;
  mia_whisper* parent = nullptr;
  int n_clones = 0;

  LinearW conv1, conv2;
  float* enc_pos = nullptr;
  std::vector<EncBlockW> enc;
  LNW ln_post;
  void* tok_emb = nullptr;
  void* tok_emb_f = nullptr;
  float* emb_c1 = nullptr;
  float* emb_c2 = nullptr;
  uint32_t* emb_qw = nullptr;
  float* emb_qst = nullptr;
  int q_bits = 0;
  int use_packed = 0;
  float* dec_pos = nullptr;
  std::vector<DecBlockW> dec;
  LNW dec_ln;

  int cap_B = 0, cur_B = 0;
  int Tpad = 0;
  void* mel_pad = nullptr;
  void* conv1_out = nullptr;
  float* x = nullptr;
  void* h = nullptr;
  void* qk = nullptr;
  void* vt = nullptr;
  void* att = nullptr;
  void* g = nullptr;
  void* feat = nullptr;
  void* cross_k = nullptr;
  void* cross_v = nullptr;

  void* self_k = nullptr;
  void* self_v = nullptr;
  float* dx = nullptr;
  void* dh = nullptr;
  void* dq = nullptr;
  void* da = nullptr;
  void* dg = nullptr;
  float* partial = nullptr;
  int weight_sharing = 0;
  float* enc_part = nullptr;
  float* enc_stat = nullptr;
  float* dstat = nullptr;
  float* logits = nullptr;
  int32_t* tokens = nullptr;
  int32_t* n_gen = nullptr;
  int32_t* finished = nullptr;
  int32_t* last_ts = nullptr;
  int32_t* out_n = nullptr;
  float* sum_logprob = nullptr;
  int32_t* n_logprob = nullptr;
  float* no_speech = nullptr;
  uint32_t* suppress_bits = nullptr;
  float* uniforms = nullptr;
  DecClip clip{};
  int32_t* out_tokens = nullptr;
  float* out_avg = nullptr;
  hipGraphExec_t step_graph = nullptr;
  hipGraphExec_t step_graph_n = nullptr;
  DecodeParams graph_params{};
  bool graph_valid = false;

  hipStream_t enc_stream = nullptr;
  hipEvent_t ev_enc_begin = nullptr, ev_enc_end = nullptr;

  void* win_dev = nullptr;
  void* win_host = nullptr;
  int win_cap = 0;
  hipEvent_t ev_win = nullptr;

  int debug_flags = 0;
  float* trace = nullptr;
  int32_t* trace_clips = nullptr;
  int trace_n = 0;
  std::vector<int32_t> trace_clip_ids;
};

struct EncStreamScope {
  mia_whisper* w; hipStream_t saved; bool on;
  explicit EncStreamScope(mia_whisper* w_) : w(w_), saved(w_->ctx->stream), on(w_->enc_stream != nullptr) {
    if (!on) return;
    (void)hipEventRecord(w->ev_enc_begin, saved);
    (void)hipStreamWaitEvent(w->enc_stream, w->ev_enc_begin, 0);
    w->ctx->stream = w->enc_stream;
  }
  ~EncStreamScope() {
    if (!on) return;
    (void)hipEventRecord(w->ev_enc_end, w->enc_stream);
    w->ctx->stream = saved;
    (void)hipStreamWaitEvent(saved, w->ev_enc_end, 0);
  }
};

int whisper_reserve(mia_whisper* w, int B);
int whisper_encode_from_padded_mel(mia_whisper* w, int B);
int whisper_decode(mia_whisper* w, const mia_decode_opts* o, int32_t* tokens, int32_t* n_tokens, float* avg_logprob,
                   float* no_speech_prob, HostIo& io);
size_t mia_logmel_scratch_bytes(int B, int64_t n_out, int n_mels);
size_t mia_logmel_direct_scratch_bytes(int B, int64_t n_out);
int mia_logmel_device(mia_ctx* ctx, const float* pcm_dev, const int64_t* offs_host, int B, int n_mels, int window_kind,
                      int64_t pad_right, int64_t n_out, void* out_dev, int out_dtype, bool channel_major,
                      int64_t clip_stride, int64_t row_stride, int64_t col_stride, int64_t row_off, void* scratch);
```

mlx-swift-audio_amd/csrc/whisper_decode.hip:

```cpp
#include <algorithm>
#include <cmath>
#include <cstdlib>
#include <vector>

#include "decode.h"

namespace {

int pick_split(int K, int want) {
  for (int s = want; s > 1; --s) if (K % (32 * s) == 0) return s;
  return 1;
}

struct AlignHook {
  float* qk = nullptr;
  const int32_t* head_slot = nullptr;
  int n_slots = 0;
  const int32_t* n_tok = nullptr;
  float* probs = nullptr;
  int eot = 0;
};

__global__ __launch_bounds__(256) void align_token_prob(const float* __restrict__ logits, const int32_t* __restrict__ tokens, int32_t* __restrict__ pos_arr,
                                                        const int32_t* __restrict__ n_tok, float* __restrict__ probs, int V, int n_ctx, int eot) {
// ... 49 lines not shown
    SkinnyArgs a{A, lda, (const uint16_t*)lw.wf, use_bias ? lw.b : nullptr, out, ldo, ck, cv, w->clip.pos, B, lw.N, lw.K, S, act, D, H, C};
    a.out_frag = out_frag;
    a.w_keep = mode == SK_OUTF32 ? p.keep_vocab : p.keep_layers;
    if (stat_in) { a.ss_in = stat_in; a.ss_tiles = D / 16; a.ss_dim = D; a.eps = 1e-5f; a.c1 = c1 ? c1 : lw.c1; a.c2 = c2 ? c2 : lw.c2; a.rs_scale = lw.ln_rs; }
    if (mode == SK_RESID) { a.xres = w->dx; a.nw = next_ln->gc; a.ss_out = stat_out; }
    if (p.packed) return dec_launch_skinny_q(w, a, lw.qw, lw.qst, p.packed, mode, s);
    return dec_launch_skinny(w, a, mode, s);
  };
  const int S_d = p.packed ? pick_split(D / 4, 2) : pick_split(D, 2), S_4d = p.packed ? pick_split(D, 4) : pick_split(4 * D, 4);
  const bool fused_ln = D % 32 == 0 && D <= 2048 && w->dec[0].qkv.c1 != nullptr && !p.split_ln && !p.packed;
  float* st_a = w->dstat;
  float* st_b = w->dstat + (size_t)(D / 16) * w->cap_B * 2;
  if (hook || !dec_head_is_split(p)) dec_launch_embed_ln(w, w->dec[0].attn_ln, s);
  for (int l = 0; l < p.L; ++l) {
    const DecBlockW& b = w->dec[l];
    uint16_t* sk = (uint16_t*)w->self_k + (size_t)l * w->cap_B * C * D;
    uint16_t* sv = (uint16_t*)w->self_v + (size_t)l * w->cap_B * C * D;
    const uint16_t* xk = (const uint16_t*)w->cross_k + (size_t)l * w->cap_B * T * D;
    const uint16_t* xv = (const uint16_t*)w->cross_v + (size_t)l * w->cap_B * T * D;
    const LNW& next_ln = l + 1 < p.L ? w->dec[l + 1].attn_ln : w->dec_ln;
    if (fused_ln) {
      if (skinny(dh, D, b.qkv, true, w->dq, D, 1, MIA_ACT_NONE, SK_QKV, sk, sv)) return -1;
      if (dec_launch_attention(w, w->dq, sk, sv, w->da, 0, C, s, nullptr, nullptr, 0, 0, p.self_nt != 0)) return -1;
      if (skinny((const uint16_t*)w->da, D, b.out, true, w->dh, D, 1, MIA_ACT_NONE, SK_RESID, nullptr, nullptr, 0, nullptr, &b.cross_ln, st_a)) return -1;
      if (skinny(dh, D, b.cq, true, w->dq, D, 1, MIA_ACT_NONE, SK_OUT16, nullptr, nullptr, 0, st_a)) return -1;
      if (dec_launch_attention(w, w->dq, xk, xv, w->da, T, T, s, hook ? hook->qk : nullptr, hook ? hook->head_slot + (size_t)l * H : nullptr,
                               hook ? hook->n_slots : 0, C)) return -1;
      if (skinny((const uint16_t*)w->da, D, b.cout, true, w->dh, D, 1, MIA_ACT_NONE, SK_RESID, nullptr, nullptr, 0, nullptr, &b.mlp_ln, st_b)) return -1;
      if (skinny(dh, D, b.mlp1, true, w->dg, 4 * D, 1, MIA_ACT_GELU, SK_OUT16, nullptr, nullptr, 1, st_b)) return -1;
      if (skinny((const uint16_t*)w->dg, 4 * D, b.mlp2, false, w->partial, 0, S_4d, MIA_ACT_NONE, SK_PARTIAL)) return -1;
      dec_launch_reduce_ln(w, S_4d, b.mlp2.b, next_ln, s);
      continue;
    }
    if (skinny(dh, D, b.qkv, true, w->dq, D, 1, MIA_ACT_NONE, SK_QKV, sk, sv)) return -1;
    if (dec_launch_attention(w, w->dq, sk, sv, w->da, 0, C, s, nullptr, nullptr, 0, 0, p.self_nt != 0)) return -1;
    if (skinny((const uint16_t*)w->da, D, b.out, false, w->partial, 0, S_d, MIA_ACT_NONE, SK_PARTIAL)) return -1;
    dec_launch_reduce_ln(w, S_d, b.out.b, b.cross_ln, s);
    if (skinny(dh, D, b.cq, true, w->dq, D, 1, MIA_ACT_NONE, SK_OUT16)) return -1;
    if (dec_launch_attention(w, w->dq, xk, xv, w->da, T, T, s, hook ? hook->qk : nullptr, hook ? hook->head_slot + (size_t)l * H : nullptr,
                             hook ? hook->n_slots : 0, C)) return -1;
    if (skinny((const uint16_t*)w->da, D, b.cout, false, w->partial, 0, S_d, MIA_ACT_NONE, SK_PARTIAL)) return -1;
    dec_launch_reduce_ln(w, S_d, b.cout.b, b.mlp_ln, s);
    if (skinny(dh, D, b.mlp1, true, w->dg, 4 * D, 1, MIA_ACT_GELU, SK_OUT16, nullptr, nullptr, 1)) return -1;
    if (skinny((const uint16_t*)w->dg, 4 * D, b.mlp2, false, w->partial, 0, S_4d, MIA_ACT_NONE, SK_PARTIAL)) return -1;
    dec_launch_reduce_ln(w, S_4d, b.mlp2.b, next_ln, s);
  }
  {
    LinearW e; e.w = w->tok_emb; e.wf = w->tok_emb_f; e.N = p.V; e.K = D; e.c1 = w->emb_c1; e.c2 = w->emb_c2; e.qw = w->emb_qw; e.qst = w->emb_qst;
    if (skinny(dh, D, e, false, w->logits, p.V, 1, MIA_ACT_NONE, SK_OUTF32)) return -1;
  }
  if (p.trace && !hook && dec_launch_trace(w, s)) return -1;
  if (hook) {
    hipLaunchKernelGGL(align_token_prob, dim3(B), dim3(256), 0, s, w->logits, w->tokens, w->clip.pos, hook->n_tok, hook->probs, p.V, C, hook->eot);
    return hipGetLastError() == hipSuccess ? 0 : -1;
  }
  if (dec_launch_head(w, w->last_ts, p, s)) return -1;
  return hipGetLastError() == hipSuccess ? 0 : -1;
}

}

int whisper_decode(mia_whisper* w, const mia_decode_opts* o, int32_t* tokens, int32_t* n_tokens, float* avg_logprob,
                   float* no_speech_prob, HostIo& io) {
  mia_ctx* ctx = w->ctx;
  const mia_whisper_dims& d = w->dims;
  MIA_CHECK_ARG(ctx, w->cur_B > 0, "decode: no audio features (call mia_whisper_encode first)");
  MIA_CHECK_ARG(ctx, o && o->initial_tokens && o->n_initial > 0, "decode: initial_tokens required");
  MIA_CHECK_ARG(ctx, o->max_tokens > 0 && o->max_tokens <= d.n_text_ctx, "decode: max_tokens must be in 1..n_text_ctx");
  MIA_CHECK_ARG(ctx, o->n_initial < o->max_tokens, "decode: initial sequence (%d) leaves no room under max_tokens (%d)", o->n_initial, o->max_tokens);
  MIA_CHECK_ARG(ctx, o->eot >= 0 && o->eot < d.n_vocab && o->no_speech >= 0 && o->no_speech < d.n_vocab &&
                         o->timestamp_begin > 0 && o->timestamp_begin <= d.n_vocab && o->no_timestamps >= 0 && o->no_timestamps < d.n_vocab,
                "decode: special token ids out of range");
  MIA_CHECK_ARG(ctx, o->n_suppress >= 0 && o->n_blank >= 0 && (o->n_suppress == 0 || o->suppress_ids) && (o->n_blank == 0 || o->blank_ids), "decode: bad suppress tables");
  MIA_CHECK_ARG(ctx, HostIo::valid(io.mem()), "decode: bad mem");
  MIA_HIP(ctx, hipSetDevice(ctx->device));
  hipStream_t s = ctx->stream;
  const int B = w->cur_B, C = d.n_text_ctx, V = d.n_vocab;

  DecodeParams p{};
  p.B = B; p.V = V; p.D = d.n_text_state; p.H = d.n_text_head; p.L = d.n_text_layer; p.n_ctx = C;
  p.eot = o->eot; p.no_speech = o->no_speech; p.no_timestamps = o->no_timestamps; p.timestamp_begin = o->timestamp_begin;
  p.timestamps = o->timestamps ? 1 : 0; p.max_tokens = o->max_tokens;
  p.max_initial_ts = o->max_initial_timestamp_index; p.max_new_tokens = o->max_new_tokens;
  p.trace = w->trace ? 1 : 0; p.head_single = (w->debug_flags & 2) ? 1 : 0; p.split_ln = (w->debug_flags & 4) ? 1 : 0;
  p.packed = w->use_packed ? w->q_bits : 0;
  const bool resident = dec_cache_policy(w, p);
  if (w->trace)
    for (int i = 0; i < w->trace_n; ++i) MIA_CHECK_ARG(ctx, w->trace_clip_ids[i] < w->cur_B, "decode: traced clip %d is not in this batch of %d", w->trace_clip_ids[i], w->cur_B);

  std::vector<int32_t> n_init(B), sot_idx(B), fin(B, 0);
  std::vector<float> temp(B);
  int total_steps = 0; bool any_sampling = false;
  {
    std::vector<int32_t> init((size_t)B * C, 0);
    for (int b = 0; b < B; ++b) {
      const int ni = (o->per_clip_initial && o->n_initial_per_clip) ? o->n_initial_per_clip[b] : o->n_initial;
      MIA_CHECK_ARG(ctx, ni > 0 && ni <= o->n_initial && ni < o->max_tokens, "decode: clip %d: bad initial length %d", b, ni);
      n_init[b] = ni;
      sot_idx[b] = o->sot_index_per_clip ? o->sot_index_per_clip[b] : o->sot_index;
      MIA_CHECK_ARG(ctx, sot_idx[b] >= 0 && sot_idx[b] < ni, "decode: clip %d: sot_index out of range", b);
      temp[b] = o->clip_temperature ? o->clip_temperature[b] : o->temperature;
      MIA_CHECK_ARG(ctx, temp[b] >= 0.0f, "decode: negative temperature");
      if (temp[b] > 0.0f) any_sampling = true;
      if (o->clip_active && !o->clip_active[b]) fin[b] = 1;
      for (int i = 0; i < ni; ++i) {
        const int32_t t = o->per_clip_initial ? o->initial_tokens[(size_t)b * o->n_initial + i] : o->initial_tokens[i];
        if (t < 0 || t >= V) return mia_fail(ctx, MIA_ERR_INVALID_ARGUMENT, "decode: initial token %d out of vocabulary", t);
        init[(size_t)b * C + i] = t;
      }
      int cap = p.max_tokens - ni;
      if (p.max_new_tokens > 0 && p.max_new_tokens < cap) cap = p.max_new_tokens;
      if (!fin[b]) total_steps = std::max(total_steps, ni + cap - 1);
    }
    MIA_CHECK_ARG(ctx, !any_sampling || o->uniforms, "decode: temperature > 0 needs caller-provided uniforms [B][max_tokens]");
    const int nw = (V + 31) / 32;
    std::vector<uint32_t> bits((size_t)2 * nw, 0u);
    auto setbit = [&](int set, int id) { if (id >= 0 && id < V) bits[(size_t)set * nw + (id >> 5)] |= 1u << (id & 31); };
    for (int i = 0; i < o->n_suppress; ++i) { setbit(0, o->suppress_ids[i]); setbit(1, o->suppress_ids[i]); }
    for (int i = 0; i < o->n_blank; ++i) setbit(1, o->blank_ids[i]);
    setbit(1, o->eot);
    io.table(init.data(), w->tokens, init.size() * 4);
    io.table(bits.data(), w->suppress_bits, bits.size() * 4);
    io.table(n_init.data(), w->clip.n_init, (size_t)B * 4);
    io.table(sot_idx.data(), w->clip.sot_idx, (size_t)B * 4);
    io.table(temp.data(), w->clip.temp, (size_t)B * 4);
    io.table(fin.data(), w->finished, (size_t)B * 4);
    if (any_sampling) {
      for (int b = 0; b < B; ++b) io.table(o->uniforms + (size_t)b * o->max_tokens, w->uniforms + (size_t)b * C, (size_t)o->max_tokens * 4);
    }
    if (int rc = io.finish()) return rc;
  }
  p.greedy = any_sampling ? 0 : 1;
  MIA_HIP(ctx, hipMemsetAsync(w->n_gen, 0, (size_t)B * 4, s));
  MIA_HIP(ctx, hipMemsetAsync(w->last_ts, 0, (size_t)B * 4, s));
  MIA_HIP(ctx, hipMemsetAsync(w->sum_logprob, 0, (size_t)B * 4, s));
  MIA_HIP(ctx, hipMemsetAsync(w->n_logprob, 0, (size_t)B * 4, s));
  MIA_HIP(ctx, hipMemsetAsync(w->no_speech, 0, (size_t)B * 4, s));
  MIA_HIP(ctx, hipMemsetAsync(w->clip.pos, 0, (size_t)B * 4, s));

  const bool no_graph = (w->debug_flags & 1) != 0;
  constexpr int DEC_GRAPH_STEPS = 8;
  if (!no_graph && (!w->graph_valid || memcmp(&w->graph_params, &p, sizeof(p)) != 0)) {
    if (w->step_graph) { (void)hipGraphExecDestroy(w->step_graph); w->step_graph = nullptr; }
    if (w->step_graph_n) { (void)hipGraphExecDestroy(w->step_graph_n); w->step_graph_n = nullptr; }
    auto capture = [&](int n_steps, hipGraphExec_t* exec) -> int {
      hipGraph_t graph = nullptr;
      MIA_HIP(ctx, hipStreamBeginCapture(s, hipStreamCaptureModeThreadLocal));
      int erc = 0;
      for (int i = 0; i < n_steps && erc == 0; ++i) erc = enqueue_step(w, p);
      hipError_t ce = hipStreamEndCapture(s, &graph);
      if (erc != 0 || ce != hipSuccess || !graph) {
        if (graph) (void)hipGraphDestroy(graph);
        return mia_fail(ctx, MIA_ERR_DEVICE, "decode: step graph capture failed (%s)", hipGetErrorString(ce));
      }
      hipError_t ie = hipGraphInstantiate(exec, graph, nullptr, nullptr, 0);
      (void)hipGraphDestroy(graph);
      if (ie != hipSuccess) return mia_fail(ctx, MIA_ERR_DEVICE, "decode: hipGraphInstantiate failed (%s)", hipGetErrorString(ie));
      return MIA_OK;
    };
    if (int rc = capture(1, &w->step_graph)) return rc;
    if (int rc = capture(DEC_GRAPH_STEPS, &w->step_graph_n)) return rc;
    w->graph_params = p;
    w->graph_valid = true;
  }

  if (dec_head_is_split(p)) dec_launch_embed_ln(w, w->dec[0].attn_ln, s);
  int prof_rec = mia_prof_begin(ctx, MIA_PROF_DECODE, 0.0);
  const int prof_kept = resident ? mia_prof_begin(ctx, MIA_PROF_DECODE_KEPT, 0.0) : -1;
  int steps_run = 0;
  const int min_init = *std::min_element(n_init.begin(), n_init.end());
  for (int step = 0; step < total_steps;) {
    int n = 1;
    if (no_graph) { if (enqueue_step(w, p) != 0) return mia_fail(ctx, MIA_ERR_DEVICE, "decode: step launch failed"); }
    else if (total_steps - step >= DEC_GRAPH_STEPS) { n = DEC_GRAPH_STEPS; MIA_HIP(ctx, hipGraphLaunch(w->step_graph_n, s)); }
    else MIA_HIP(ctx, hipGraphLaunch(w->step_graph, s));
    step += n;
    steps_run += n;
    if (step > min_init && (step & 15) == 0 && step < total_steps) {
      io.fetch(fin.data(), w->finished, (size_t)B * 4);
      if (int rc = io.finish()) return rc;
      bool all = true;
      for (int b = 0; b < B; ++b) all = all && fin[b];
      if (all) break;
    }
  }
  if (prof_kept >= 0) { ctx->prof[prof_kept].work = steps_run; mia_prof_end(ctx, prof_kept); }
  if (prof_rec >= 0) { ctx->prof[prof_rec].work = steps_run; mia_prof_end(ctx, prof_rec); }
  dec_launch_finalize(w, w->out_n, p, s);
  MIA_HIP(ctx, hipGetLastError());
  const hipMemcpyKind kind = io.to_caller();
  if (tokens) io.check(hipMemcpyAsync(tokens, w->out_tokens, (size_t)B * p.max_tokens * 4, kind, s));
  if (n_tokens) io.check(hipMemcpyAsync(n_tokens, w->out_n, (size_t)B * 4, kind, s));
  if (avg_logprob) io.check(hipMemcpyAsync(avg_logprob, w->out_avg, (size_t)B * 4, kind, s));
  if (no_speech_prob) io.check(hipMemcpyAsync(no_speech_prob, w->no_speech, (size_t)B * 4, kind, s));
  return io.finish();
}

namespace {

__global__ __launch_bounds__(256) void align_softmax_rows(float* __restrict__ qk, const int32_t* __restrict__ n_tok, const int32_t* __restrict__ n_fr,
                                                          int n_slots, int n_ctx, int T) {
  __shared__ float red[8];
  const int tok = blockIdx.x, slot = blockIdx.y, b = blockIdx.z;
  if (tok >= n_tok[b]) return;
  const int F = n_fr[b];
  float* row = qk + (((int64_t)b * n_slots + slot) * n_ctx + tok) * T;
  const int tid = threadIdx.x, lane = tid & 63, wave = tid >> 6;
  float m = -INFINITY;
  for (int i = tid; i < F; i += 256) m = fmaxf(m, row[i]);
  m = wave_max(m);
  if (lane == 0) red[wave] = m;
  __syncthreads();
  m = fmaxf(fmaxf(red[0], red[1]), fmaxf(red[2], red[3]));
  float sum = 0.f;
  for (int i = tid; i < F; i += 256) sum += expf(row[i] - m);
  sum = wave_sum(sum);
  if (lane == 0) red[4 + wave] = sum;
  __syncthreads();
  sum = (red[4] + red[5]) + (red[6] + red[7]);
  for (int i = tid; i < F; i += 256) row[i] = expf(row[i] - m) / sum;
}

__global__ __launch_bounds__(256) void align_standardize(float* __restrict__ qk, const int32_t* __restrict__ n_tok, const int32_t* __restrict__ n_fr,
                                                         int n_slots, int n_ctx, int T) {
  const int f = blockIdx.x * 256 + threadIdx.x, slot = blockIdx.y, b = blockIdx.z;
  if (f >= n_fr[b]) return;
  const int n = n_tok[b];
  float* col = qk + ((int64_t)b * n_slots + slot) * n_ctx * T + f;
  float s = 0.f;
  for (int t = 0; t < n; ++t) s += col[(int64_t)t * T];
  const float mean = s / (float)n;
  float q = 0.f;
  for (int t = 0; t < n; ++t) { const float d = col[(int64_t)t * T] - mean; q += d * d; }
  const float inv = 1.0f / sqrtf(q / (float)n + 1e-8f);
  for (int t = 0; t < n; ++t) col[(int64_t)t * T] = (col[(int64_t)t * T] - mean) * inv;
}

__device__ __forceinline__ void cswap(float& a, float& b) { const float lo = fminf(a, b), hi = fmaxf(a, b); a = lo; b = hi; }
__device__ __forceinline__ float median7(float v0, float v1, float v2, float v3, float v4, float v5, float v6) {
  cswap(v0, v6); cswap(v2, v3); cswap(v4, v5);
  cswap(v0, v2); cswap(v1, v4); cswap(v3, v6);
  cswap(v0, v1); cswap(v2, v5); cswap(v3, v4);
  cswap(v1, v2); cswap(v4, v6);
  cswap(v2, v3); cswap(v4, v5);
  cswap(v1, v2); cswap(v3, v4); cswap(v5, v6);
  return v3;
}

__global__ __launch_bounds__(256) void align_median_mean(const float* __restrict__ qk, const int32_t* __restrict__ n_tok, const int32_t* __restrict__ n_fr,
// ... 43 lines not shown
  std::reverse(ti.begin(), ti.end()); std::reverse(tj.begin(), tj.end());
}

}

extern "C" int mia_whisper_align(mia_whisper* w, const int32_t* tokens, int stride, const int32_t* n_tokens, const int32_t* heads, int n_heads,
                                 const int32_t* num_frames, int row_start, int eot, float* token_probs, int32_t* text_idx, int32_t* time_idx,
                                 int32_t* path_len, int path_cap, float* matrix) {
  if (!w) return MIA_ERR_MODEL_NOT_LOADED;
  mia_ctx* ctx = w->ctx;
  const mia_whisper_dims& d = w->dims;
  const int B = w->cur_B, C = d.n_text_ctx, T = d.n_audio_ctx, H = d.n_text_head, L = d.n_text_layer;
  MIA_CHECK_ARG(ctx, B > 0, "align: no audio features (call mia_whisper_encode first)");
  MIA_CHECK_ARG(ctx, tokens && n_tokens && heads && num_frames && token_probs && text_idx && time_idx && path_len, "align: null argument");
  MIA_CHECK_ARG(ctx, n_heads > 0 && n_heads <= 64 && stride > 0 && stride <= C && row_start >= 0 && eot > 0 && eot <= d.n_vocab && path_cap > 0, "align: bad sizes");
  MIA_HIP(ctx, hipSetDevice(ctx->device));
  hipStream_t s = ctx->stream;
  std::vector<int32_t> slot((size_t)L * H, -1), ntok(B), nfr(B), init((size_t)B * C, 0);
  for (int i = 0; i < n_heads; ++i) {
    const int l = heads[2 * i], h = heads[2 * i + 1];
    MIA_CHECK_ARG(ctx, l >= 0 && l < L && h >= 0 && h < H, "align: alignment head (%d, %d) out of range", l, h);
    slot[(size_t)l * H + h] = i;
  }
  int max_tok = 0;
  for (int b = 0; b < B; ++b) {
    ntok[b] = n_tokens[b];
    MIA_CHECK_ARG(ctx, ntok[b] >= 2 && ntok[b] <= stride && row_start < ntok[b] - 1, "align: clip %d: token count %d out of range", b, ntok[b]);
    nfr[b] = num_frames[b] / 2;
    MIA_CHECK_ARG(ctx, nfr[b] >= 2 && nfr[b] <= T, "align: clip %d: frame count out of range", b);
    for (int i = 0; i < ntok[b]; ++i) {
      const int32_t t = tokens[(size_t)b * stride + i];
      MIA_CHECK_ARG(ctx, t >= 0 && t < d.n_vocab, "align: token out of vocabulary");
      init[(size_t)b * C + i] = t;
    }
    max_tok = std::max(max_tok, ntok[b]);
  }
  const size_t n_qk = (size_t)B * n_heads * C * T, n_cost = (size_t)B * C * T;
  auto al = [](size_t n) { return (n + 63) / 64 * 64; };
  const size_t floats = al(n_qk) + al(n_cost) + al((size_t)B * C) + al((size_t)L * H) + 2 * al(B);
  float* ws = (float*)mia_workspace(ctx, floats * 4);
  if (!ws) return MIA_ERR_OUT_OF_MEMORY;
  float* d_qk = ws; float* d_cost = d_qk + al(n_qk); float* d_probs = d_cost + al(n_cost);
  int32_t* d_slot = (int32_t*)(d_probs + al((size_t)B * C)); int32_t* d_ntok = d_slot + al((size_t)L * H); int32_t* d_nfr = d_ntok + al(B);
  MIA_HIP(ctx, hipMemcpyAsync(w->tokens, init.data(), init.size() * 4, hipMemcpyHostToDevice, s));
  MIA_HIP(ctx, hipMemcpyAsync(d_slot, slot.data(), slot.size() * 4, hipMemcpyHostToDevice, s));
  MIA_HIP(ctx, hipMemcpyAsync(d_ntok, ntok.data(), (size_t)B * 4, hipMemcpyHostToDevice, s));
  MIA_HIP(ctx, hipMemcpyAsync(d_nfr, nfr.data(), (size_t)B * 4, hipMemcpyHostToDevice, s));
  MIA_HIP(ctx, hipMemsetAsync(w->clip.pos, 0, (size_t)B * 4, s));
  MIA_HIP(ctx, hipMemsetAsync(d_probs, 0, (size_t)B * C * 4, s));
  MIA_HIP(ctx, hipStreamSynchronize(s));

  DecodeParams p{};
  p.B = B; p.V = d.n_vocab; p.D = d.n_text_state; p.H = H; p.L = L; p.n_ctx = C; p.packed = w->use_packed ? w->q_bits : 0;
  dec_cache_policy(w, p);
  AlignHook hook; hook.qk = d_qk; hook.head_slot = d_slot; hook.n_slots = n_heads; hook.n_tok = d_ntok; hook.probs = d_probs; hook.eot = eot;
  for (int step = 0; step < max_tok; ++step)
    if (enqueue_step(w, p, &hook) != 0) return mia_fail(ctx, MIA_ERR_DEVICE, "align: step launch failed");
  hipLaunchKernelGGL(align_softmax_rows, dim3(max_tok, n_heads, B), dim3(256), 0, s, d_qk, d_ntok, d_nfr, n_heads, C, T);
  hipLaunchKernelGGL(align_standardize, dim3((T + 255) / 256, n_heads, B), dim3(256), 0, s, d_qk, d_ntok, d_nfr, n_heads, C, T);
  hipLaunchKernelGGL(align_median_mean, dim3((T + 255) / 256, max_tok, B), dim3(256), 0, s, d_qk, d_ntok, d_nfr, n_heads, C, T, d_cost);
  MIA_HIP(ctx, hipGetLastError());
  std::vector<float> cost(n_cost);
  MIA_HIP(ctx, hipMemcpyAsync(cost.data(), d_cost, n_cost * 4, hipMemcpyDeviceToHost, s));
  std::vector<float> probs((size_t)B * C);
  MIA_HIP(ctx, hipMemcpyAsync(probs.data(), d_probs, probs.size() * 4, hipMemcpyDeviceToHost, s));
  MIA_HIP(ctx, hipStreamSynchronize(s));
  std::vector<int32_t> ti, tj;
  for (int b = 0; b < B; ++b) {
    for (int i = 0; i < stride; ++i) token_probs[(size_t)b * stride + i] = i < C ? probs[(size_t)b * C + i] : 0.f;
    const int N = ntok[b] - 1 - row_start;
    dtw_host(cost.data() + ((size_t)b * C + row_start) * T, N, nfr[b], T, ti, tj);
    if ((int)ti.size() > path_cap) return mia_fail(ctx, MIA_ERR_INVALID_ARGUMENT, "align: path_cap %d too small (need %zu)", path_cap, ti.size());
    path_len[b] = (int32_t)ti.size();
    for (size_t i = 0; i < ti.size(); ++i) { text_idx[(size_t)b * path_cap + i] = ti[i]; time_idx[(size_t)b * path_cap + i] = tj[i]; }
    if (matrix)
      for (int t = 0; t < ntok[b]; ++t)
        for (int f2 = 0; f2 < T; ++f2) matrix[((size_t)b * stride + t) * T + f2] = f2 < nfr[b] ? -cost[((size_t)b * C + t) * T + f2] : 0.f;
  }
  return MIA_OK;
}

extern "C" int mia_whisper_set_debug(mia_whisper* w, int flags) {
  if (!w) return MIA_ERR_MODEL_NOT_LOADED;
  MIA_CHECK_ARG(w->ctx, flags >= 0 && (flags & ~23) == 0, "set_debug: flags must be a combination of 1, 2, 4 and 16 (got %d)", flags);
  w->debug_flags = flags;
  return MIA_OK;
}

extern "C" int mia_whisper_trace_logits(mia_whisper* w, const int32_t* clips, int n_clips) {
  if (!w) return MIA_ERR_MODEL_NOT_LOADED;
  mia_ctx* ctx = w->ctx;
  MIA_CHECK_ARG(ctx, n_clips >= 0 && n_clips <= 8 && (n_clips == 0 || clips), "trace_logits: 0..8 clips");
  MIA_HIP(ctx, hipSetDevice(ctx->device));
  MIA_HIP(ctx, hipStreamSynchronize(ctx->stream));
  w->graph_valid = false;
  if (w->trace) { (void)hipFree(w->trace); w->trace = nullptr; }
  if (w->trace_clips) { (void)hipFree(w->trace_clips); w->trace_clips = nullptr; }
  w->trace_n = 0;
  w->trace_clip_ids.clear();
  if (n_clips == 0) return MIA_OK;
  for (int i = 0; i < n_clips; ++i) MIA_CHECK_ARG(ctx, clips[i] >= 0, "trace_logits: negative clip index");
  const size_t bytes = (size_t)n_clips * w->dims.n_text_ctx * w->dims.n_vocab * sizeof(float);
  if (hipMalloc((void**)&w->trace, bytes) != hipSuccess) { w->trace = nullptr; return mia_fail(ctx, MIA_ERR_OUT_OF_MEMORY, "trace_logits: hipMalloc(%zu) failed", bytes); }
  if (hipMalloc((void**)&w->trace_clips, (size_t)n_clips * 4) != hipSuccess) { (void)hipFree(w->trace); w->trace = nullptr; w->trace_clips = nullptr; return mia_fail(ctx, MIA_ERR_OUT_OF_MEMORY, "trace_logits: hipMalloc failed"); }
  MIA_HIP(ctx, hipMemsetAsync(w->trace, 0xff, bytes, ctx->stream));
  MIA_HIP(ctx, hipMemcpyAsync(w->trace_clips, clips, (size_t)n_clips * 4, hipMemcpyHostToDevice, ctx->stream));
  MIA_HIP(ctx, hipStreamSynchronize(ctx->stream));
  w->trace_n = n_clips;
  w->trace_clip_ids.assign(clips, clips + n_clips);
  return MIA_OK;
}

extern "C" int mia_whisper_read_logit_trace(mia_whisper* w, int slot, int first_pos, int n_pos, float* out) {
  if (!w) return MIA_ERR_MODEL_NOT_LOADED;
  mia_ctx* ctx = w->ctx;
  MIA_CHECK_ARG(ctx, w->trace && slot >= 0 && slot < w->trace_n, "read_logit_trace: no trace for slot %d", slot);
  MIA_CHECK_ARG(ctx, out && first_pos >= 0 && n_pos > 0 && first_pos + n_pos <= w->dims.n_text_ctx, "read_logit_trace: bad position range");
  MIA_HIP(ctx, hipSetDevice(ctx->device));
  const size_t V = w->dims.n_vocab;
  MIA_HIP(ctx, hipMemcpyAsync(out, w->trace + ((size_t)slot * w->dims.n_text_ctx + first_pos) * V, (size_t)n_pos * V * 4, hipMemcpyDeviceToHost, ctx->stream));
  MIA_HIP(ctx, hipStreamSynchronize(ctx->stream));
  return MIA_OK;
}

extern "C" int mia_whisper_decode_greedy(mia_whisper* w, const mia_decode_opts* opts, int32_t* tokens, int32_t* n_tokens,
                                         float* avg_logprob, float* no_speech_prob, int mem) {
  if (!w) return MIA_ERR_MODEL_NOT_LOADED;
  HostIo io(w->ctx, mem);
  return whisper_decode(w, opts, tokens, n_tokens, avg_logprob, no_speech_prob, io);
}

static __global__ void lang_kernel(const float* __restrict__ logits, int V, int start, int n, int32_t* __restrict__ idx, float* __restrict__ prob) {
  const int b = blockIdx.x;
  const float* lg = logits + (int64_t)b * V + start;
  if (threadIdx.x == 0) {
    float m = -INFINITY; int mi = 0;
    for (int i = 0; i < n; ++i) if (lg[i] > m) { m = lg[i]; mi = i; }
    float s = 0.f;
    for (int i = 0; i < n; ++i) s += __expf(lg[i] - m);
    idx[b] = mi;
    prob[b] = 1.0f / s;
  }
}

extern "C" int mia_whisper_detect_language(mia_whisper* w, int32_t sot, int32_t n_languages, int32_t* lang_idx, float* prob) {
  if (!w) return MIA_ERR_MODEL_NOT_LOADED;
  mia_ctx* ctx = w->ctx;
  const mia_whisper_dims& d = w->dims;
  MIA_CHECK_ARG(ctx, w->cur_B > 0, "detect_language: no audio features (call mia_whisper_encode first)");
  MIA_CHECK_ARG(ctx, lang_idx && prob, "detect_language: null outputs");
  MIA_CHECK_ARG(ctx, sot >= 0 && n_languages > 0 && sot + 1 + n_languages <= d.n_vocab, "detect_language: token range out of vocabulary");
  int32_t init = sot;
  mia_decode_opts o{};
  o.initial_tokens = &init; o.n_initial = 1; o.sot_index = 0;
  o.eot = sot > 0 ? sot - 1 : 0; o.no_speech = 0; o.no_timestamps = 0; o.timestamp_begin = d.n_vocab; o.timestamps = 0;
  o.max_tokens = 2; o.max_initial_timestamp_index = 50;
  HostIo io = HostIo::device(ctx);
  int rc = whisper_decode(w, &o, nullptr, nullptr, nullptr, nullptr, io);
  if (rc != MIA_OK) return rc;
  const int B = w->cur_B;
  hipLaunchKernelGGL(lang_kernel, dim3(B), dim3(64), 0, ctx->stream, w->logits, d.n_vocab, sot + 1, n_languages, w->out_n, w->out_avg);
  MIA_HIP(ctx, hipMemcpyAsync(lang_idx, w->out_n, (size_t)B * 4, hipMemcpyDeviceToHost, ctx->stream));
  MIA_HIP(ctx, hipMemcpyAsync(prob, w->out_avg, (size_t)B * 4, hipMemcpyDeviceToHost, ctx->stream));
  MIA_HIP(ctx, hipStreamSynchronize(ctx->stream));
  return MIA_OK;
}

// ... 61 lines not shown
```

mlx-swift-audio_amd/csrc/whisper_encode.hip:

```cpp
#include <cstdlib>

#include "whisper.h"

namespace {

int gemm(mia_whisper* w, GemmArgs g, int cls = MIA_PROF_ENC_GEMM) {
  g.variant = w->gemm_variant;
  if (const char* e = mia_gemm_check(g)) return mia_fail(w->ctx, MIA_ERR_INVALID_ARGUMENT, "%s", e);
  const int rec = mia_prof_begin(w->ctx, cls, 2.0 * g.M * (double)g.N * g.K * (g.batch > 0 ? g.batch : 1));
  const int rc = mia_gemm_launch(g, w->dtype, w->ctx->stream);
  mia_prof_end(w->ctx, rec);
  if (rc != 0) return mia_fail(w->ctx, MIA_ERR_DEVICE, "gemm launch failed");
  return MIA_OK;
}

int norm(mia_whisper* w, const LNW& ln, void* out, int M, int D) {
  const int rec = mia_prof_begin(w->ctx, MIA_PROF_ENC_NORM, (double)M * D * 6.0);
  const int rc = mia_norm_launch(w->x, D, ln.g, ln.b, out, D, M, D, 1e-5f, false, w->dtype, w->ctx->stream);
  mia_prof_end(w->ctx, rec);
  if (rc) return mia_fail(w->ctx, MIA_ERR_DEVICE, "norm launch failed");
  return MIA_OK;
}

}

int whisper_reserve(mia_whisper* w, int B) {
  if (B <= w->cap_B) return MIA_OK;
  MIA_HIP(w->ctx, hipStreamSynchronize(w->ctx->stream));
  w->graph_valid = false;
  const mia_whisper_dims& d = w->dims;
  const size_t D = d.n_audio_state, T = d.n_audio_ctx, H = d.n_audio_head, L = d.n_text_layer;
  const size_t M = (size_t)B * T;
  const int Tpad = (int)align_up(T, 64);
  std::vector<void*> fresh;
  bool ok = true;
  auto get = [&](size_t bytes, bool zero) -> void* {
    if (!ok) return nullptr;
    void* q = nullptr;
    if (hipMalloc(&q, bytes ? bytes : 16) != hipSuccess) { ok = false; mia_fail(w->ctx, MIA_ERR_OUT_OF_MEMORY, "hipMalloc(%zu) failed for batch buffers", bytes); return nullptr; }
    fresh.push_back(q);
    if (zero && hipMemsetAsync(q, 0, bytes, w->ctx->stream) != hipSuccess) { ok = false; mia_fail(w->ctx, MIA_ERR_DEVICE, "memset failed"); }
    return q;
  };
  mia_whisper n = *w;
#define A(p, bytes, zero) n.p = (decltype(n.p))get((bytes), (zero))
  A(mel_pad, ((size_t)B * (2 * T + 2) * d.n_mels + 256) * 2, true);
  A(conv1_out, (size_t)B * (2 * T + 1) * D * 2, true);
  A(x, M * D * 4, false);
  A(h, M * D * 2, false);
  A(qk, M * 2 * D * 2, false);
  A(vt, (size_t)B * H * 64 * Tpad * 2, true);
  A(att, M * D * 2, false);
  A(g, M * 4 * D * 2, false);
  A(feat, M * D * 2, false);
  A(enc_part, M * (D / 64 + 1) * 2 * 4, false);
  A(enc_stat, M * 2 * 4, false);
  A(cross_k, L * M * D * 2, false);
  A(cross_v, L * M * D * 2, false);
  const size_t C = d.n_text_ctx, V = d.n_vocab;
  A(self_k, L * B * C * D * 2, true);
  A(self_v, L * B * C * D * 2, true);
  A(dx, (size_t)B * D * 4, false);
  const size_t B32 = align_up((size_t)B, 32);
  A(dh, B32 * D * 2, true);
  A(dq, (size_t)B * D * 2, false);
  A(da, B32 * D * 2, true);
  A(dg, B32 * 4 * D * 2, true);
  A(partial, (size_t)16 * B * D * 4, false);
  A(dstat, (size_t)2 * ((D + 15) / 16) * B * 2 * 4, true);
  A(logits, (size_t)B * V * 4, false);
  A(tokens, (size_t)B * C * 4, true);
  A(n_gen, (size_t)B * 4, true);
  A(finished, (size_t)B * 4, true);
  A(last_ts, (size_t)B * 4, true);
  A(out_n, (size_t)B * 4, true);
  A(sum_logprob, (size_t)B * 4, true);
  A(n_logprob, (size_t)B * 4, true);
  A(no_speech, (size_t)B * 4, true);
  A(uniforms, (size_t)B * C * 4, true);
  A(out_tokens, (size_t)B * C * 4, true);
  A(out_avg, (size_t)B * 4, true);
  A(clip.pos, (size_t)B * 4, true);
  A(clip.n_init, (size_t)B * 4, true);
  A(clip.sot_idx, (size_t)B * 4, true);
  A(clip.temp, (size_t)B * 4, true);
#undef A
  if (ok && hipStreamSynchronize(w->ctx->stream) != hipSuccess) { ok = false; mia_fail(w->ctx, MIA_ERR_DEVICE, "stream sync failed"); }
  if (!ok) {
    for (void* q : fresh) (void)hipFree(q);
    return w->ctx->err.find("hipMalloc") != std::string::npos ? MIA_ERR_OUT_OF_MEMORY : MIA_ERR_DEVICE;
  }
  if (!w->suppress_bits) {
    void* q = nullptr;
    const size_t bytes = 2 * ((V + 31) / 32) * 4;
    if (hipMalloc(&q, bytes) != hipSuccess) { for (void* f : fresh) (void)hipFree(f); return mia_fail(w->ctx, MIA_ERR_OUT_OF_MEMORY, "hipMalloc(%zu) failed", bytes); }
    (void)hipMemsetAsync(q, 0, bytes, w->ctx->stream);
    w->allocs.push_back(q);
    w->suppress_bits = (uint32_t*)q;
  }
  w->mel_pad = n.mel_pad; w->conv1_out = n.conv1_out; w->x = n.x; w->h = n.h; w->qk = n.qk; w->vt = n.vt; w->att = n.att; w->g = n.g;
  w->feat = n.feat; w->enc_part = n.enc_part; w->enc_stat = n.enc_stat; w->cross_k = n.cross_k; w->cross_v = n.cross_v; w->self_k = n.self_k; w->self_v = n.self_v; w->dx = n.dx; w->dh = n.dh;
  w->dq = n.dq; w->da = n.da; w->dg = n.dg; w->partial = n.partial; w->dstat = n.dstat; w->logits = n.logits; w->tokens = n.tokens; w->n_gen = n.n_gen;
  w->finished = n.finished; w->last_ts = n.last_ts; w->out_n = n.out_n; w->sum_logprob = n.sum_logprob; w->n_logprob = n.n_logprob;
  w->no_speech = n.no_speech; w->uniforms = n.uniforms; w->out_tokens = n.out_tokens; w->out_avg = n.out_avg; w->clip = n.clip;
  for (void* q : w->batch_allocs) (void)hipFree(q);
  w->batch_allocs.swap(fresh);
  w->Tpad = Tpad;
  w->cap_B = B;
  return MIA_OK;
}

int whisper_encode_from_padded_mel(mia_whisper* w, int B) {
  const mia_whisper_dims& d = w->dims;
  const int D = d.n_audio_state, T = d.n_audio_ctx, H = d.n_audio_head, M = B * T;
  hipStream_t s = w->ctx->stream;
  int rc;
  {
    GemmArgs g;
    g.A = w->mel_pad; g.lda = d.n_mels; g.strideA = (int64_t)(2 * T + 2) * d.n_mels;
    g.W = w->conv1.w; g.bias = w->conv1.b; g.act = MIA_ACT_GELU;
    g.C = (uint16_t*)w->conv1_out + D; g.ldc = D; g.strideC = (int64_t)(2 * T + 1) * D;
    g.M = 2 * T; g.N = D; g.K = w->kpad_conv1; g.batch = B;
    if ((rc = gemm(w, g)) != MIA_OK) return rc;
  }
  {
    GemmArgs g;
    g.A = w->conv1_out; g.lda = 2 * D; g.strideA = (int64_t)(2 * T + 1) * D;
    g.W = w->conv2.w; g.bias = w->conv2.b; g.act = MIA_ACT_GELU;
    g.R = w->enc_pos; g.ldr = D; g.strideR = 0;
    g.C = w->x; g.ldc = D; g.strideC = (int64_t)T * D; g.out_f32 = 1;
    g.M = T; g.N = D; g.K = 3 * D; g.batch = B;
    if ((rc = gemm(w, g)) != MIA_OK) return rc;
  }
  for (int l = 0; l < d.n_audio_layer; ++l) {
    const EncBlockW& b = w->enc[l];
    if ((rc = norm(w, b.attn_ln, w->h, M, D)) != MIA_OK) return rc;
    {
      GemmArgs g;
      g.A = w->h; g.lda = D; g.W = b.qkv.w; g.bias = b.qkv.b;
      g.C = w->qk; g.ldc = 2 * D; g.C2 = w->vt;
      g.M = M; g.N = 3 * D; g.K = D; g.epi = MIA_EPI_QKV_VT; g.T = T; g.H = H; g.Tpad = w->Tpad;
      if ((rc = gemm(w, g)) != MIA_OK) return rc;
    }
    if (const char* e = mia_enc_attention_check(B, T, H, w->Tpad, 2 * D, D)) return mia_fail(w->ctx, MIA_ERR_INVALID_ARGUMENT, "%s", e);
    {
      const int rec = mia_prof_begin(w->ctx, MIA_PROF_ENC_ATTN, 4.0 * B * H * (double)T * T * 64);
      const int arc = mia_enc_attention_launch(w->qk, 2 * D, w->vt, w->att, D, B, T, H, w->Tpad, w->dtype, s);
      mia_prof_end(w->ctx, rec);
      if (arc) return mia_fail(w->ctx, MIA_ERR_DEVICE, "attention launch failed");
    }
    {
      GemmArgs go, g1;
      go.A = w->att; go.lda = D; go.W = b.out.w; go.bias = b.out.b;
      go.R = w->x; go.ldr = D; go.C = w->x; go.ldc = D; go.out_f32 = 1;
      go.M = M; go.N = D; go.K = D; go.variant = w->gemm_variant;
      g1.A = w->h; g1.lda = D; g1.W = b.mlp1.w; g1.bias = b.mlp1.b; g1.act = MIA_ACT_GELU;
      g1.C = w->g; g1.ldc = 4 * D; g1.M = M; g1.N = 4 * D; g1.K = D; g1.variant = w->gemm_variant;
      GemmArgs fo = go, f1 = g1;
      fo.ln_gamma = b.mlp_ln.gc; fo.ln_out = w->h; fo.ln_ld = D; fo.ln_part = w->enc_part;
      f1.ln_stat = w->enc_stat; f1.ln_c1 = b.mlp1.c1; f1.bias = b.mlp1.c2;
      const bool carry = b.mlp1.c1 && b.mlp1.c2 && mia_gemm_ln_ok(fo) && mia_gemm_ln_ok(f1);
      if ((rc = gemm(w, carry ? fo : go)) != MIA_OK) return rc;
      if (carry) {
        const int rec = mia_prof_begin(w->ctx, MIA_PROF_ENC_NORM, (double)M * (D / 64) * 8.0);
        const int frc = mia_ln_finalize_launch(w->enc_part, D / 64, D, 1e-5f, w->enc_stat, M, s, b.mlp1.ln_rs);
        mia_prof_end(w->ctx, rec);
        if (frc) return mia_fail(w->ctx, MIA_ERR_DEVICE, "ln finalize launch failed");
      } else if ((rc = norm(w, b.mlp_ln, w->h, M, D)) != MIA_OK) return rc;
      if ((rc = gemm(w, carry ? f1 : g1)) != MIA_OK) return rc;
    }
    {
      GemmArgs g;
      g.A = w->g; g.lda = 4 * D; g.W = b.mlp2.w; g.bias = b.mlp2.b;
      g.R = w->x; g.ldr = D; g.C = w->x; g.ldc = D; g.out_f32 = 1;
      g.M = M; g.N = D; g.K = 4 * D;
      if ((rc = gemm(w, g)) != MIA_OK) return rc;
    }
  }
  if ((rc = norm(w, w->ln_post, w->feat, M, D)) != MIA_OK) return rc;
  for (int l = 0; l < d.n_text_layer; ++l) {
    const DecBlockW& b = w->dec[l];
    const size_t off = (size_t)l * w->cap_B * T * D;
    for (int kv = 0; kv < 2; ++kv) {
      GemmArgs g;
      g.A = w->feat; g.lda = D; g.W = kv ? b.cv.w : b.ck.w; g.bias = kv ? b.cv.b : b.ck.b;
      g.C = (uint16_t*)(kv ? w->cross_v : w->cross_k) + off;
// ... 69 lines not shown
```

mlx-swift-audio_amd/ops.py:

```python
from __future__ import annotations

import ctypes as C

import numpy as np

from . import _lib
from ._abi import ConvGemmDesc, SkinnyDesc
from . import audio as _audio


def to16(a: np.ndarray, dtype: int) -> np.ndarray:
    return np.ascontiguousarray(a, np.float32).astype(np.float16) if dtype == _lib.F16 else _audio.f32_to_bf16(a)


def from16(a: np.ndarray, dtype: int) -> np.ndarray:
    return a.astype(np.float32) if dtype == _lib.F16 else _audio.bf16_to_f32(a)


def linear(ctx: _lib.Context, x: np.ndarray, w: np.ndarray, bias=None, residual=None, act: str | None = None,
           dtype: int = _lib.BF16, out_f32: bool = False, variant: int = 1) -> np.ndarray:
    M, K = x.shape
    N = w.shape[0]
    x16, w16 = to16(x, dtype), to16(w, dtype)
    b = None if bias is None else np.ascontiguousarray(bias, np.float32)
# ... 167 lines not shown

def _ptr(t):
    return None if t is None else t.data_ptr()


def _ld(t, ld):
    return int(ld) if ld is not None else (int(t.stride(0)) if t is not None and t.dim() == 2 else 0)


def _run(ctx, call):
    import torch
    torch.cuda.synchronize()
    try:
        ctx.check(call())
    finally:
        ctx.synchronize()


def conv1d_f32(ctx: _lib.Context, x, w, y, *, Cin: int, taps: int = 1, stride: int = 1, dil: int = 1, pad: int = 0, act: int = 0, bias=None,
               r=None, T_in: int | None = None, T_out: int | None = None, N: int | None = None, ldx: int | None = None,
               ldy: int | None = None) -> np.ndarray:
    dx, dw, dy, db, dr = _dev(x), _dev(w), _dev(y), _dev(bias), _dev(r)
    _run(ctx, lambda: ctx.lib.mia_op_conv1d_f32(ctx.h, _ptr(dx), _ld(dx, ldx), int(dx.shape[0] if T_in is None else T_in), _ptr(dw), _ptr(db),
                                                 _ptr(dr), _ptr(dy), _ld(dy, ldy), int(dy.shape[0] if T_out is None else T_out),
                                                 int(dw.shape[0] if N is None else N), int(Cin), int(taps), int(stride), int(dil), int(pad), int(act)))
    return dy.cpu().numpy()


def conv_gemm_f32(ctx: _lib.Context, phases: int = 1, **d) -> np.ndarray:
    unknown = set(d) - {n for n, _ in ConvGemmDesc._fields_}
    assert not unknown, f"not a mia_conv_gemm_desc field: {sorted(unknown)}"
    t = {k: _dev(d.get(k)) for k in _DESC_F32}
    t.update({k: _dev(d.get(k), np.int32) for k in _DESC_I32})
    desc = ConvGemmDesc()
    for name, _ in ConvGemmDesc._fields_:
        if name in t:
            setattr(desc, name, _ptr(t[name]))
        elif name in ("ldx", "ldy", "ldr"):
            setattr(desc, name, _ld(t[{"ldx": "X", "ldy": "Y", "ldr": "R"}[name]] if name != "ldr" or t["R"] is not None else t["R2"], d.get(name)))
        else:
            setattr(desc, name, d.get(name, _DESC_DEFAULTS.get(name, 0)))
    _run(ctx, lambda: ctx.lib.mia_op_conv_gemm_f32(ctx.h, C.byref(desc), int(phases)))
    return None if t["Y"] is None else t["Y"].cpu().numpy()


def attention_f32_ex(ctx: _lib.Context, q, k, v, out, B: int, T: int, H: int, scale: float = 0.125, p=None, bias_u=None, bias_v=None,
                     seq_len=None, chunk: int = 0, ldq=None, ldk=None, ldv=None, ldp=None, ldo=None, plain: bool = False) -> np.ndarray:
    dq, dk, dv, do, dp, du, dbv = _dev(q), _dev(k), _dev(v), _dev(out), _dev(p), _dev(bias_u), _dev(bias_v)
    ds = _dev(seq_len, np.int32)
    head = (ctx.h, _ptr(dq), _ld(dq, ldq), _ptr(dk), _ld(dk, ldk), _ptr(dv), _ld(dv, ldv))
    if plain:
        assert p is None and seq_len is None and not chunk
        _run(ctx, lambda: ctx.lib.mia_op_attention_f32(*head, _ptr(do), _ld(do, ldo), int(B), int(T), int(H), float(scale)))
    else:
        _run(ctx, lambda: ctx.lib.mia_op_attention_f32_ex(*head, _ptr(dp), _ld(dp, ldp), _ptr(du), _ptr(dbv), _ptr(do), _ld(do, ldo), int(B), int(T),
                                                           int(H), float(scale), _ptr(ds), int(chunk)))
    return do.cpu().numpy()


def attention_f32(ctx: _lib.Context, q, k, v, out, B: int, T: int, H: int, scale: float = 0.125, **ld) -> np.ndarray:
    return attention_f32_ex(ctx, q, k, v, out, B, T, H, scale, plain=True, **ld)




SK_OUT16, SK_OUTF32, SK_PARTIAL, SK_QKV, SK_SWIGLU, SK_RESID = range(6)
_SKINNY_PTRS = ("A", "W", "wfrag", "stfrag", "bias", "out", "xres", "nw", "ss_out", "ss_in")


def quant_repack(codes: np.ndarray, scales: np.ndarray, biases: np.ndarray, bits: int, scale_dtype: int, compute_dtype: int):
    lib = _lib.load()
    codes, scales, biases = np.ascontiguousarray(codes, np.uint32), np.ascontiguousarray(scales), np.ascontiguousarray(biases)
    N, K = codes.shape[0], codes.shape[1] * (32 // bits)
    tiles = (N + 15) // 16
    wf = np.zeros((tiles, K // 128, bits // 4, 64, 4), np.uint32)
    st = np.zeros((tiles, K // 128, 16, 4), np.float32)
    rc = lib.mia_quant_repack(codes.ctypes.data, scales.ctypes.data, biases.ctypes.data, N, K, int(bits), int(scale_dtype), int(compute_dtype),
                              wf.ctypes.data, st.ctypes.data)
    if rc != 0:
        raise _lib.MiaError(rc, "quant_repack: bad argument")
    return wf, st


def skinny_gemm(ctx: _lib.Context, **d) -> None:
    lib = ctx.lib
    unknown = set(d) - {n for n, _ in SkinnyDesc._fields_}
    assert not unknown, f"not a mia_skinny_desc field: {sorted(unknown)}"
    desc = SkinnyDesc()
    for name, _ in SkinnyDesc._fields_:
        v = d.get(name)
        if name in _SKINNY_PTRS:
            assert v is None or v.is_cuda, "device tensors only"
            setattr(desc, name, _ptr(v))
        elif name == "lda":
            desc.lda = _ld(d.get("A"), v)
        elif name == "ldo":
            desc.ldo = _ld(d.get("out"), v)
        else:
            setattr(desc, name, {"S": 1, "rs_scale": 1.0}.get(name, 0) if v is None else v)
    _run(ctx, lambda: lib.mia_op_skinny_gemm(ctx.h, C.byref(desc)))
```

Measured before the change: 4907 audio-sec/s.

## Add LDS-staged vocab GEMM and cached per-clip head state for decode

The vocabulary projection (OUTF32 skinny GEMM) gains an LDS-staged kernel. It is picked automatically when the weights fit and the tile count is large relative to the CU count; otherwise the old fring kernel runs. The split decode head now keeps a compact per-clip HeadState (position, last tokens, last timestamp, finished) that the final kernel updates. Partial blocks read that one struct instead of gathering from several buffers, and suppress-mask words are prefetched into registers. A test ABI for forcing the vocab variant, plus a debug flag for the old state loader, is added; the extra state must stay consistent with the token buffers.

```diff
diff --git a/include/mia.h b/include/mia.h
--- a/include/mia.h
+++ b/include/mia.h
@@ -138,6 +138,7 @@
   int32_t M_cap;
 } mia_skinny_desc;
 int mia_op_skinny_gemm(mia_ctx* ctx, const mia_skinny_desc* d);
+int mia_op_skinny_gemm_variant(mia_ctx* ctx, const mia_skinny_desc* d, int variant);
 
 typedef struct {
   int32_t n_mels, n_audio_ctx, n_audio_state, n_audio_head, n_audio_layer;
diff --git a/mlx-swift-audio_amd/_abi.py b/mlx-swift-audio_amd/_abi.py
--- a/mlx-swift-audio_amd/_abi.py
+++ b/mlx-swift-audio_amd/_abi.py
@@ -207,6 +207,7 @@
     "mia_op_kvq_attention": (i32, [vp, vp, vp, vp, vp] + [i32] * 6),
     "mia_op_lm_prompt_attention": (i32, [vp, vp, vp, vp, vp] + [i32] * 6),
     "mia_op_skinny_gemm": (i32, [vp, P(SkinnyDesc)]),
+    "mia_op_skinny_gemm_variant": (i32, [vp, P(SkinnyDesc), i32]),
     "mia_whisper_load": (vp, [vp, P(WhisperDims), TV, i32, i32]),
     "mia_whisper_free": (None, [vp]),
     "mia_whisper_clone": (vp, [vp, vp]),
diff --git a/mlx-swift-audio_amd/csrc/decode.h b/mlx-swift-audio_amd/csrc/decode.h
--- a/mlx-swift-audio_amd/csrc/decode.h
+++ b/mlx-swift-audio_amd/csrc/decode.h
@@ -13,4 +13,5 @@
 bool dec_head_is_split(const DecodeParams& p);
 int dec_launch_trace(mia_whisper* w, hipStream_t s);
 int dec_launch_head(mia_whisper* w, int32_t* last_ts, const DecodeParams& p, hipStream_t s);
+int dec_launch_head_state_init(mia_whisper* w, hipStream_t s);
 int dec_launch_finalize(mia_whisper* w, int32_t* out_n, const DecodeParams& p, hipStream_t s);
diff --git a/mlx-swift-audio_amd/csrc/decode_kernels.hip b/mlx-swift-audio_amd/csrc/decode_kernels.hip
--- a/mlx-swift-audio_amd/csrc/decode_kernels.hip
+++ b/mlx-swift-audio_amd/csrc/decode_kernels.hip
@@ -235,6 +235,7 @@
   const uint32_t* suppress;
   const float* uniforms;
   DecClip clip;
+  HeadState* state;
 };
 
 constexpr int HEAD_NPT = 52;
@@ -260,24 +261,24 @@
   int ts_floor;
   int max_first;
   int num_gen, cur_len;
+  bool probe;
 };
-__device__ __forceinline__ HeadRule head_rule(const HeadBufs& hb, const DecodeParams& p, int b) {
+__device__ __forceinline__ HeadRule head_rule_from(const HeadState& st, const DecodeParams& p) {
   HeadRule r{};
-  const int pos = hb.clip.pos[b], n_initial = hb.clip.n_init[b], sot_index = hb.clip.sot_idx[b];
+  const int pos = st.pos, n_initial = st.n_init;
   r.cur_len = pos + 1;
   const bool generating = r.cur_len >= n_initial;
-  r.active = !(generating && hb.finished[b]) && (generating || pos == sot_index);
+  r.active = !(generating && st.finished) && (generating || pos == st.sot_idx);
+  r.probe = r.active && pos == st.sot_idx;
   r.decide = generating;
   r.num_gen = r.cur_len - n_initial;
   r.max_first = p.V;
   if (r.active && r.decide && p.timestamps) {
-    const int32_t* toks = hb.tokens + (int64_t)b * p.n_ctx;
     const int tsb = p.timestamp_begin;
-    const int last = toks[r.cur_len - 1];
-    const bool last_was_ts = r.num_gen >= 1 && last >= tsb;
-    const bool penult_was_ts = r.num_gen < 2 || toks[r.cur_len - 2] >= tsb;
+    const bool last_was_ts = r.num_gen >= 1 && st.last >= tsb;
+    const bool penult_was_ts = r.num_gen < 2 || st.penult >= tsb;
     if (last_was_ts) { if (penult_was_ts) r.sup_ts_all = true; else r.sup_text_below_eot = true; }
-    const int lt = hb.last_ts[b];
+    const int lt = st.last_ts;
     if (lt > 0) r.ts_floor = penult_was_ts ? lt + 1 : lt;
     if (r.num_gen == 0) {
       r.sup_below_tsb = true;
@@ -288,10 +289,22 @@
   }
   return r;
 }
-
-__device__ __forceinline__ bool head_masked(const HeadRule& r, const DecodeParams& p, const uint32_t* bits, int i) {
+__device__ __forceinline__ HeadState head_state_load(const HeadBufs& hb, const DecodeParams& p, int b) {
+  HeadState st{};
+  st.pos = hb.clip.pos[b]; st.n_init = hb.clip.n_init[b]; st.sot_idx = hb.clip.sot_idx[b]; st.finished = hb.finished[b];
+  if (st.pos + 1 >= st.n_init && p.timestamps) {
+    const int32_t* toks = hb.tokens + (int64_t)b * p.n_ctx;
+    st.last = toks[st.pos];
+    if (st.pos >= 1) st.penult = toks[st.pos - 1];
+    st.last_ts = hb.last_ts[b];
+  }
+  return st;
+}
+__device__ __forceinline__ HeadRule head_rule(const HeadBufs& hb, const DecodeParams& p, int b) { return head_rule_from(head_state_load(hb, p, b), p); }
+
+__device__ __forceinline__ bool head_masked(const HeadRule& r, const DecodeParams& p, uint32_t word, int i) {
   const int tsb = p.timestamp_begin;
-  if ((bits[i >> 5] >> (i & 31)) & 1u) return true;
+  if ((word >> (i & 31)) & 1u) return true;
   if (p.timestamps) {
     if (i == p.no_timestamps) return true;
     if (r.sup_ts_all && i >= tsb) return true;
@@ -314,15 +327,25 @@
 }
 
 template <int NTH, int NPT>
-__device__ __forceinline__ HeadPart head_reduce(const float (&x)[NPT], int base, const HeadRule& r, const HeadBufs& hb, const DecodeParams& p,
-                                                HeadKept<NPT>& okA) {
+__device__ __forceinline__ void head_sup_load(uint32_t (&w0)[NPT], uint32_t (&w1)[NPT], const uint32_t* suppress, int base, int V) {
+  const int nw = (V + 31) / 32;
+#pragma unroll
+  for (int u = 0; u < NPT; ++u) {
+    const int i = base + (int)threadIdx.x + NTH * u;
+    w0[u] = i < V ? suppress[i >> 5] : 0u;
+    w1[u] = i < V ? suppress[nw + (i >> 5)] : 0u;
+  }
+}
+
+template <int NTH, int NPT, typename Sup>
+__device__ __forceinline__ HeadPart head_reduce(const float (&x)[NPT], int base, const HeadRule& r, const DecodeParams& p,
+                                                HeadKept<NPT>& okA, Sup sup) {
   constexpr int NWV = NTH / 64;
   __shared__ float shf[NWV][4];
   __shared__ float sha[NWV][2];
   __shared__ int shai[NWV][2];
   const int tid = threadIdx.x, lane = tid & 63, wave = tid >> 6;
   const int V = p.V, tsb = p.timestamp_begin;
-  const uint32_t* bits = hb.suppress + (r.num_gen == 0 ? (V + 31) / 32 : 0);
   float mx_text = -INFINITY, mx_ts = -INFINITY;
   ArgMax bA{-INFINITY, HEAD_NONE}, bB{-INFINITY, HEAD_NONE};
   okA = 0;
@@ -331,7 +354,7 @@
     const int i = base + tid + NTH * u;
     if (i >= V) continue;
     if (i >= tsb) mx_ts = fmaxf(mx_ts, x[u]); else mx_text = fmaxf(mx_text, x[u]);
-    if (r.decide && !head_masked(r, p, bits, i)) {
+    if (r.decide && !head_masked(r, p, sup(u, i), i)) {
       okA |= (HeadKept<NPT>)1 << u;
       bA = amax(bA, ArgMax{x[u], i});
       if (i >= tsb) bB = amax(bB, ArgMax{x[u], i});
@@ -386,16 +409,18 @@
 }
 
 __device__ __forceinline__ void head_probe(const HeadBufs& hb, const DecodeParams& p, int b, const HeadRule& r, float lse) {
-  if (r.active && r.cur_len - 1 == hb.clip.sot_idx[b]) hb.no_speech[b] = __expf(hb.logits[(int64_t)b * p.V + p.no_speech] - lse);
-}
-
-__device__ __forceinline__ int head_commit(const HeadBufs& hb, const DecodeParams& p, int b, const HeadRule& r, const HeadPick& k, int next) {
+  if (r.probe) hb.no_speech[b] = __expf(hb.logits[(int64_t)b * p.V + p.no_speech] - lse);
+}
+
+__device__ __forceinline__ int head_commit(const HeadBufs& hb, const DecodeParams& p, int b, const HeadRule& r, const HeadPick& k, int next,
+                                           HeadState* st = nullptr, const float* x_next = nullptr) {
   const int pos = r.cur_len - 1, n_initial = r.cur_len - r.num_gen;
   int newpos = -1;
   if (!r.decide) newpos = pos + 1;
   else if (r.active) {
     if (next != p.eot) {
-      hb.sum_logprob[b] += k.all_masked ? __int_as_float(0x7fc00000) : (hb.logits[(int64_t)b * p.V + next] - k.best.v) - __logf(k.fsum);
+      const float xn = k.all_masked ? 0.f : x_next ? *x_next : hb.logits[(int64_t)b * p.V + next];
+      hb.sum_logprob[b] += k.all_masked ? __int_as_float(0x7fc00000) : (xn - k.best.v) - __logf(k.fsum);
       hb.n_logprob[b] += 1;
     }
     hb.tokens[(int64_t)b * p.n_ctx + r.cur_len] = next;
@@ -403,10 +428,16 @@
     if (next > p.timestamp_begin) hb.last_ts[b] = next;
     int cap = p.max_tokens - n_initial;
     if (p.max_new_tokens > 0 && p.max_new_tokens < cap) cap = p.max_new_tokens;
-    if (next == p.eot || r.num_gen + 1 >= cap) hb.finished[b] = 1;
+    const bool fin = next == p.eot || r.num_gen + 1 >= cap;
+    if (fin) hb.finished[b] = 1;
     else newpos = pos + 1;
-  }
-  if (newpos >= 0) hb.clip.pos[b] = newpos;
+    if (st) {
+      st->penult = st->last; st->last = next;
+      if (next > p.timestamp_begin) st->last_ts = next;
+      if (fin) st->finished = 1;
+    }
+  }
+  if (newpos >= 0) { hb.clip.pos[b] = newpos; if (st) st->pos = newpos; }
   return newpos;
 }
 
@@ -424,7 +455,8 @@
   float x[HEAD_NPT];
   head_load<1024, HEAD_NPT>(x, hb.logits + (int64_t)b * p.V, 0, p.V);
   HeadKept<HEAD_NPT> okA;
-  const HeadPart m = head_reduce<1024, HEAD_NPT>(x, 0, r, hb, p, okA);
+  const uint32_t* bits = hb.suppress + (r.num_gen == 0 ? (p.V + 31) / 32 : 0);
+  const HeadPart m = head_reduce<1024, HEAD_NPT>(x, 0, r, p, okA, [&](int, int i) { return bits[i >> 5]; });
   const HeadPick k = head_decide(r, m);
   if (tid == 0) head_probe(hb, p, b, r, k.lse);
   int next = k.next;
@@ -483,11 +515,14 @@
   const int k = blockIdx.x, b = blockIdx.y;
   const int base = k * (256 * HEAD_NPT2);
   float x[HEAD_NPT2];
+  uint32_t w0[HEAD_NPT2], w1[HEAD_NPT2];
   head_load<256, HEAD_NPT2>(x, hb.logits + (int64_t)b * p.V, base, p.V);
-  const HeadRule r = head_rule(hb, p, b);
+  head_sup_load<256, HEAD_NPT2>(w0, w1, hb.suppress, base, p.V);
+  const HeadRule r = head_rule_from(p.head_loader ? head_state_load(hb, p, b) : hb.state[b], p);
   if (!r.active) return;
+  const bool first = r.num_gen == 0;
   HeadKept<HEAD_NPT2> okA;
-  const HeadPart part = head_reduce<256, HEAD_NPT2>(x, base, r, hb, p, okA);
+  const HeadPart part = head_reduce<256, HEAD_NPT2>(x, base, r, p, okA, [&](int u, int) { return first ? w1[u] : w0[u]; });
   if (threadIdx.x == 0) parts[b * HEAD_SPLIT + k] = part;
 }
 
@@ -495,15 +530,18 @@
 
 template <typename T>
 __global__ __launch_bounds__(256) void dec_head_final(HeadBufs hb, DecodeParams p, const HeadPart* __restrict__ parts, NextEmbed ne) {
-  __shared__ int s_newpos;
+  __shared__ int s_newpos, s_tok;
   __shared__ float sh[4];
   const int b = blockIdx.x, tid = threadIdx.x;
   float mx_text = -INFINITY, mx_ts = -INFINITY, s_all = 0.f, s_ts = 0.f, fA = 0.f, fB = 0.f;
   ArgMax bA{-INFINITY, HEAD_NONE}, bB{-INFINITY, HEAD_NONE};
-  const HeadRule r = head_rule(hb, p, b);
+  HeadPart me{-INFINITY, -INFINITY, 0.f, 0.f, -INFINITY, -INFINITY, 0.f, 0.f, HEAD_NONE, HEAD_NONE};
+  if (tid < HEAD_SPLIT) me = parts[b * HEAD_SPLIT + tid];
+  HeadState st = p.head_loader ? head_state_load(hb, p, b) : hb.state[b];
+  const HeadRule r = head_rule_from(st, p);
+  const int fpos = st.pos + 1 < p.n_ctx ? st.pos + 1 : p.n_ctx - 1;
+  const int ftok = hb.tokens[(int64_t)b * p.n_ctx + fpos];
   if (tid < 64 && r.active) {
-    HeadPart me{-INFINITY, -INFINITY, 0.f, 0.f, -INFINITY, -INFINITY, 0.f, 0.f, HEAD_NONE, HEAD_NONE};
-    if (tid < HEAD_SPLIT) me = parts[b * HEAD_SPLIT + tid];
     mx_text = wave_max(me.mx_text); mx_ts = wave_max(me.mx_ts);
     bA = wave_amax(ArgMax{me.bAv, me.bAi}); bB = wave_amax(ArgMax{me.bBv, me.bBi});
     const float mx_all = fmaxf(mx_text, mx_ts);
@@ -516,13 +554,15 @@
   if (tid == 0) {
     const HeadPick k = head_decide(r, HeadPart{mx_text, mx_ts, s_all, s_ts, bA.v, bB.v, fA, fB, bA.i, bB.i});
     head_probe(hb, p, b, r, k.lse);
-    s_newpos = head_commit(hb, p, b, r, k, k.next);
+    s_newpos = head_commit(hb, p, b, r, k, k.next, &st, &k.best.v);
+    s_tok = r.decide ? k.next : ftok;
+    hb.state[b] = st;
   }
   __syncthreads();
   const int np_ = s_newpos;
   if (np_ < 0 || np_ >= p.n_ctx) return;
   const int D = ne.D, nv = D >> 2;
-  const int tok = hb.tokens[(int64_t)b * p.n_ctx + np_];
+  const int tok = s_tok;
   const uint16_t* e = ne.emb + (int64_t)tok * D;
   const float* pe = ne.pos_emb + (int64_t)np_ * D;
   float* xr = ne.x + (int64_t)b * D;
@@ -610,9 +650,20 @@
   return 0;
 }
 
+__global__ void dec_head_state_init(HeadState* __restrict__ st, const int32_t* __restrict__ n_init, const int32_t* __restrict__ sot_idx,
+                                    const int32_t* __restrict__ finished, int B) {
+  const int b = blockIdx.x * blockDim.x + threadIdx.x;
+  if (b < B) st[b] = HeadState{0, n_init[b], sot_idx[b], finished[b], 0, 0, 0, 0};
+}
+
+int dec_launch_head_state_init(mia_whisper* w, hipStream_t s) {
+  hipLaunchKernelGGL(dec_head_state_init, dim3((w->cur_B + 63) / 64), dim3(64), 0, s, w->head_state, w->clip.n_init, w->clip.sot_idx, w->finished, w->cur_B);
+  return 0;
+}
+
 int dec_launch_head(mia_whisper* w, int32_t* last_ts, const DecodeParams& p, hipStream_t s) {
   if (p.V > 1024 * HEAD_NPT) return -1;
-  HeadBufs hb{w->logits, w->tokens, w->n_gen, w->finished, last_ts, w->sum_logprob, w->n_logprob, w->no_speech, w->suppress_bits, w->uniforms, w->clip};
+  HeadBufs hb{w->logits, w->tokens, w->n_gen, w->finished, last_ts, w->sum_logprob, w->n_logprob, w->no_speech, w->suppress_bits, w->uniforms, w->clip, w->head_state};
   if (dec_head_is_split(p)) {
     HeadPart* parts = reinterpret_cast<HeadPart*>(w->partial);
     hipLaunchKernelGGL(dec_head_partial, dim3(HEAD_SPLIT, w->cur_B), dim3(256), 0, s, hb, p, parts);
diff --git a/mlx-swift-audio_amd/csrc/ops_abi.hip b/mlx-swift-audio_amd/csrc/ops_abi.hip
--- a/mlx-swift-audio_amd/csrc/ops_abi.hip
+++ b/mlx-swift-audio_amd/csrc/ops_abi.hip
@@ -186,6 +186,30 @@
   return MIA_OK;
 }
 
+extern "C" int mia_op_skinny_gemm_variant(mia_ctx* ctx, const mia_skinny_desc* d, int variant) {
+  if (!ctx) return MIA_ERR_INVALID_ARGUMENT;
+  MIA_CHECK_ARG(ctx, d, "op_skinny_gemm_variant: null descriptor");
+  if (const char* e = skinny_abi_check(*d)) return mia_fail(ctx, MIA_ERR_INVALID_ARGUMENT, "op_skinny_gemm_variant: %s", e);
+  MIA_CHECK_ARG(ctx, d->mode == SK_OUTF32 && !d->wfrag && d->S == 1, "op_skinny_gemm_variant: mode 1 (OUTF32) on 16-bit weights only");
+  MIA_CHECK_ARG(ctx, variant == 0 || variant == 1, "op_skinny_gemm_variant: variant must be 0 or 1 (got %d)", variant);
+  MIA_CHECK_ARG(ctx, d->M > 0 && d->N > 0 && d->K > 0 && d->K % 32 == 0 && d->lda % 8 == 0 &&
+                         ((uint64_t)d->N + 15) / 16 * 16 * (uint64_t)d->K * 2 <= 0xffffffffull && ((uint64_t)d->M + 31) / 32 * 32 * (uint64_t)d->K * 2 <= 0xffffffffull,
+                "op_skinny_gemm_variant: M, N, K must be positive, K a multiple of 32, lda of 8, operands below 4 GiB");
+  MIA_CHECK_ARG(ctx, !d->ss_in || (d->nw && d->xres && d->ss_tiles > 0 && d->ss_tiles <= 128 && d->ss_dim > 0), "op_skinny_gemm_variant: carried statistics need c1 (nw), c2 (xres), 1..128 tiles");
+  MIA_HIP(ctx, hipSetDevice(ctx->device));
+  const size_t wbytes = (size_t)((d->N + 15) / 16) * 16 * d->K * 2, abytes = (size_t)((d->M + 31) / 32) * 32 * d->K * 2;
+  char* ws = (char*)mia_workspace(ctx, wbytes + abytes);
+  if (!ws) return MIA_ERR_OUT_OF_MEMORY;
+  if (dec_launch_repack_wfrag(d->W, ws, d->N, d->K, ctx->stream) || dec_launch_repack_afrag(d->A, d->lda, ws + wbytes, d->M, d->K, ctx->stream))
+    return mia_fail(ctx, MIA_ERR_DEVICE, "op_skinny_gemm_variant: fragment repack failed");
+  SkinnyArgs a{(const uint16_t*)(ws + wbytes), d->K, (const uint16_t*)ws, d->bias, d->out, d->ldo, nullptr, nullptr, nullptr, d->M, d->N, d->K, 1, MIA_ACT_NONE, 0, 0, 0};
+  a.w_keep = d->w_frag ? 1 : 0;
+  if (d->ss_in) { a.ss_in = d->ss_in; a.ss_tiles = d->ss_tiles; a.ss_dim = d->ss_dim; a.eps = d->eps; a.rs_scale = d->rs_scale; a.c1 = d->nw; a.c2 = d->xres; }
+  if (dec_launch_vocab_variant(a, d->dtype, variant, ctx->stream)) return mia_fail(ctx, MIA_ERR_INVALID_ARGUMENT, "op_skinny_gemm_variant: the launcher refused the arguments");
+  if (hipGetLastError() != hipSuccess) return mia_fail(ctx, MIA_ERR_DEVICE, "op_skinny_gemm_variant: launch failed");
+  return MIA_OK;
+}
+
 extern "C" int mia_op_attention_f32_ex(mia_ctx* ctx, const float* q, int64_t ldq, const float* k, int64_t ldk, const float* v, int64_t ldv,
                                        const float* p, int64_t ldp, const float* bias_u, const float* bias_v, float* out, int64_t ldo, int B, int T,
                                        int H, float scale, const int32_t* seq_len, int chunk) {
diff --git a/mlx-swift-audio_amd/csrc/skinny.h b/mlx-swift-audio_amd/csrc/skinny.h
--- a/mlx-swift-audio_amd/csrc/skinny.h
+++ b/mlx-swift-audio_amd/csrc/skinny.h
@@ -53,5 +53,7 @@
 
 int dec_launch_repack_wfrag(const void* src, void* dst, int N, int K, hipStream_t s);
 bool dec_wfrag_copy(const void* src, int N, int K, std::vector<void*>& allocs, hipStream_t s, void** dst);
+int dec_launch_repack_afrag(const void* src, int64_t lda, void* dst, int M, int K, hipStream_t s);
+int dec_launch_vocab_variant(const SkinnyArgs& a, int dtype, int variant, hipStream_t s);
 int skinny_gemm_launch(const SkinnyArgs& a, int mode, int dtype, hipStream_t s);
 int skinny_gemm_q_launch(const SkinnyArgs& a, const uint32_t* wfrag, const float* stfrag, int bits, int mode, int dtype, hipStream_t s, int M_cap = 0);
diff --git a/mlx-swift-audio_amd/csrc/skinny_frag.hip b/mlx-swift-audio_amd/csrc/skinny_frag.hip
--- a/mlx-swift-audio_amd/csrc/skinny_frag.hip
+++ b/mlx-swift-audio_amd/csrc/skinny_frag.hip
@@ -280,10 +280,135 @@
   else skinny_epilogue_v<T, MODE, NT>(a, acc, pre, blockIdx.x * (16 * NT), z * 32, split, lane, st);
 }
 
+constexpr int VOCAB_LDS_K = 2048;
+constexpr int VOCAB_LDS_NW = 16;
+constexpr int VOCAB_LDS_KB = 2;
+constexpr int VOCAB_LDS_MIN_TILES = 4;
+
+template <typename T, int NW, int KB>
+__global__ __launch_bounds__(64 * NW) void dec_vocab_lds(SkinnyArgs a) {
+  constexpr int MODE = SK_OUTF32;
+  __shared__ __attribute__((aligned(16))) uint16_t lds_a[VOCAB_LDS_K * 32];
+  __shared__ float st[64];
+  const int lane = threadIdx.x & 63, wave = threadIdx.x >> 6;
+  const int z = blockIdx.z;
+  LnStat<NW> lnstat;
+  lnstat.issue(a, z * 32, wave, lane);
+  const int ksteps = a.K >> 5, tiles = (a.N + 15) >> 4;
+  const WFragBuf ab(a, 0);
+  {
+    constexpr int MAXL = VOCAB_LDS_K * 4 / (64 * NW);
+    const int nchunk = a.K * 4;
+    const uint32_t a0 = (uint32_t)z * (uint32_t)a.K * 64u;
+    s16x8 v[MAXL];
+#pragma unroll
+    for (int j = 0; j < MAXL; ++j) {
+      const int c = (int)threadIdx.x + 64 * NW * j;
+      if (c < nchunk) v[j] = ab.template load<0>(a0 + 16u * (uint32_t)c);
+    }
+#pragma unroll
+    for (int j = 0; j < MAXL; ++j) {
+      const int c = (int)threadIdx.x + 64 * NW * j;
+      if (c < nchunk) *reinterpret_cast<s16x8*>(lds_a + 8 * c) = v[j];
+    }
+  }
+  lnstat.finish(a, st, lane);
+  __syncthreads();
+  const int gw = blockIdx.x * NW + wave, nwaves = gridDim.x * NW;
+  const int t_begin = (int)((int64_t)gw * tiles / nwaves), t_end = (int)((int64_t)(gw + 1) * tiles / nwaves);
+  const bool keep = a.w_keep != 0;
+  const WFragBuf wb(a);
+  const s16x8* la = reinterpret_cast<const s16x8*>(lds_a) + lane;
+  auto run = [&](auto nt_tag, int tile0) {
+    constexpr int NT = decltype(nt_tag)::value;
+    uint32_t wo[NT];
+#pragma unroll
+    for (int t = 0; t < NT; ++t) wo[t] = (uint32_t)(tile0 + t) * (uint32_t)ksteps * 1024u + 16u * (uint32_t)lane;
+    const SkinnyPre<NT> pre = skinny_prefetch<MODE, NT>(a, tile0 * 16, z * 32, lane);
+    f32x4 acc[NT][2];
+#pragma unroll
+    for (int t = 0; t < NT; ++t) { acc[t][0] = (f32x4){0.f, 0.f, 0.f, 0.f}; acc[t][1] = (f32x4){0.f, 0.f, 0.f, 0.f}; }
+    struct Batch { s16x8 w[KB][NT]; };
+    auto load_batch = [&](Batch& b, int ks) {
+      auto go = [&](auto keep_tag) {
+        constexpr int AUX = decltype(keep_tag)::value ? 0 : 2;
+#pragma unroll
+        for (int u = 0; u < KB; ++u)
+#pragma unroll
+          for (int n = 0; n < NT; ++n) b.w[u][n] = wb.template load<AUX>(wo[n] + 1024u * (uint32_t)(ks + u));
+      };
+      if (keep) go(std::true_type{}); else go(std::false_type{});
+    };
+    auto mma_batch = [&](const Batch& b, int ks) {
+#pragma unroll
+      for (int u = 0; u < KB; ++u) {
+        const s16x8 fa0 = la[(ks + u) * 128], fa1 = la[(ks + u) * 128 + 64];
+#pragma unroll
+        for (int n = 0; n < NT; ++n) {
+          acc[n][0] = T::mfma16(b.w[u][n], fa0, acc[n][0]);
+          acc[n][1] = T::mfma16(b.w[u][n], fa1, acc[n][1]);
+        }
+      }
+    };
+    const int nb = ksteps / KB;
+    int ks = 0;
+    if (nb > 0) {
+      Batch b0, b1, b2, b3;
+      load_batch(b0, 0);
+      if (nb > 1) load_batch(b1, KB);
+      if (nb > 2) load_batch(b2, 2 * KB);
+      for (int i = 0; i < nb; i += 4) {
+        if (i + 3 < nb) load_batch(b3, (i + 3) * KB);
+        mma_batch(b0, i * KB);
+        if (i + 1 >= nb) break;
+        if (i + 4 < nb) load_batch(b0, (i + 4) * KB);
+        mma_batch(b1, (i + 1) * KB);
+        if (i + 2 >= nb) break;
+        if (i + 5 < nb) load_batch(b1, (i + 5) * KB);
+        mma_batch(b2, (i + 2) * KB);
+        if (i + 3 >= nb) break;
+        if (i + 6 < nb) load_batch(b2, (i + 6) * KB);
+        mma_batch(b3, (i + 3) * KB);
+      }
+      ks = nb * KB;
+    }
+    for (; ks < ksteps; ++ks) {
+      const s16x8 fa0 = la[ks * 128], fa1 = la[ks * 128 + 64];
+#pragma unroll
+      for (int n = 0; n < NT; ++n) {
+        const s16x8 fw = wb.template load<0>(wo[n] + 1024u * (uint32_t)ks);
+        acc[n][0] = T::mfma16(fw, fa0, acc[n][0]);
+        acc[n][1] = T::mfma16(fw, fa1, acc[n][1]);
+      }
+    }
+    skinny_epilogue_v<T, MODE, NT>(a, acc, pre, tile0 * 16, z * 32, 0, lane, st);
+  };
+  for (int t = t_begin; t < t_end; ++t) run(std::integral_constant<int, 1>{}, t);
+}
+
+static bool vocab_lds_fits(const SkinnyArgs& a) { return a.S == 1 && a.K % 32 == 0 && a.K <= VOCAB_LDS_K; }
+
+static int vocab_lds_cus() {
+  static int n = 0;
+  if (n == 0) {
+    int dev = 0, v = 0;
+    if (hipGetDevice(&dev) == hipSuccess && hipDeviceGetAttribute(&v, hipDeviceAttributeMultiprocessorCount, dev) == hipSuccess && v > 0) n = v;
+    else n = 256;
+  }
+  return n;
+}
+
 template <typename T, int MODE>
-static int skinny_frag_launch_m(const SkinnyArgs& a, hipStream_t s) {
+static int skinny_frag_launch_m(const SkinnyArgs& a, hipStream_t s, int vocab_variant = -1) {
   const int tiles = (a.N + 15) / 16, zb = (a.M + 31) / 32, ksteps = a.K / 32;
   if constexpr (MODE == SK_OUTF32) {
+    const int cus = vocab_lds_cus();
+    const bool staged = vocab_variant < 0 ? vocab_lds_fits(a) && tiles >= VOCAB_LDS_MIN_TILES * cus : vocab_variant == 1 && vocab_lds_fits(a);
+    if (staged) {
+      const int grid = tiles < cus ? tiles : cus;
+      hipLaunchKernelGGL((dec_vocab_lds<T, VOCAB_LDS_NW, VOCAB_LDS_KB>), dim3(grid, 1, zb), dim3(64 * VOCAB_LDS_NW), 0, s, a);
+      return 0;
+    }
     hipLaunchKernelGGL((dec_skinny_fring<T, MODE, 4, 2, 1>), dim3((tiles + 3) / 4, a.S, zb), dim3(64), 0, s, a);
     return 0;
   } else {
@@ -310,10 +435,10 @@
 }
 
 template <typename T>
-static int skinny_frag_launch_t(const SkinnyArgs& a, int mode, hipStream_t s) {
+static int skinny_frag_launch_t(const SkinnyArgs& a, int mode, hipStream_t s, int vocab_variant = -1) {
   switch (mode) {
     case SK_OUT16: return skinny_frag_launch_m<T, SK_OUT16>(a, s);
-    case SK_OUTF32: return skinny_frag_launch_m<T, SK_OUTF32>(a, s);
+    case SK_OUTF32: return skinny_frag_launch_m<T, SK_OUTF32>(a, s, vocab_variant);
     case SK_PARTIAL: return skinny_frag_launch_m<T, SK_PARTIAL>(a, s);
     case SK_QKV: return skinny_frag_launch_m<T, SK_QKV>(a, s);
     case SK_RESID: return skinny_frag_launch_m<T, SK_RESID>(a, s);
@@ -329,3 +454,33 @@
   if (a.c1 && (!a.c2 || !a.ss_in || a.ss_tiles <= 0 || a.ss_tiles > 128 || a.ss_dim <= 0)) return -1;
   return w->dtype == MIA_F16 ? skinny_frag_launch_t<F16>(a, mode, s) : skinny_frag_launch_t<BF16>(a, mode, s);
 }
+
+template <typename T>
+__global__ __launch_bounds__(256) void repack_afrag(const uint16_t* __restrict__ src, int64_t lda, uint16_t* __restrict__ dst, int M, int K) {
+  const int64_t chunk = (int64_t)blockIdx.x * 256 + threadIdx.x;
+  const int ksteps = K >> 5;
+  const int64_t total = (int64_t)((M + 31) >> 5) * ksteps * 128;
+  if (chunk >= total) return;
+  const int lane = (int)(chunk & 63), mt = (int)((chunk >> 6) & 1);
+  const int64_t zk = chunk >> 7;
+  const int kstep = (int)(zk % ksteps), zb = (int)(zk / ksteps);
+  const int m = zb * 32 + mt * 16 + (lane & 15), k = kstep * 32 + 8 * (lane >> 4);
+  s16x8 v = (s16x8){0, 0, 0, 0, 0, 0, 0, 0};
+  if (m < M) v = *reinterpret_cast<const s16x8*>(src + (int64_t)m * lda + k);
+  *reinterpret_cast<s16x8*>(dst + chunk * 8) = v;
+}
+
+int dec_launch_repack_afrag(const void* src, int64_t lda, void* dst, int M, int K, hipStream_t s) {
+  if (M <= 0 || K <= 0 || K % 32 != 0 || lda % 8 != 0) return -1;
+  const int64_t total = (int64_t)((M + 31) / 32) * (K / 32) * 128;
+  hipLaunchKernelGGL(repack_afrag<BF16>, dim3((unsigned)((total + 255) / 256)), dim3(256), 0, s, (const uint16_t*)src, lda, (uint16_t*)dst, M, K);
+  return hipGetLastError() == hipSuccess ? 0 : -1;
+}
+
+int dec_launch_vocab_variant(const SkinnyArgs& a, int dtype, int variant, hipStream_t s) {
+  if (!a.A || !a.W || !a.out || a.M <= 0 || a.N <= 0 || a.S != 1 || a.K <= 0 || a.K % 32 != 0) return -1;
+  if (variant != 0 && variant != 1) return -1;
+  if (a.c1 && (!a.c2 || !a.ss_in || a.ss_tiles <= 0 || a.ss_tiles > 128 || a.ss_dim <= 0)) return -1;
+  if ((uint64_t)((a.N + 15) / 16) * 16 * (uint64_t)a.K * 2 > 0xffffffffull || (uint64_t)((a.M + 31) / 32) * 32 * (uint64_t)a.K * 2 > 0xffffffffull) return -1;
+  return dtype == MIA_F16 ? skinny_frag_launch_t<F16>(a, SK_OUTF32, s, variant) : skinny_frag_launch_t<BF16>(a, SK_OUTF32, s, variant);
+}
diff --git a/mlx-swift-audio_amd/csrc/whisper.h b/mlx-swift-audio_amd/csrc/whisper.h
--- a/mlx-swift-audio_amd/csrc/whisper.h
+++ b/mlx-swift-audio_amd/csrc/whisper.h
@@ -45,6 +45,12 @@
   float* temp;
 };
 
+struct alignas(32) HeadState {
+  int32_t pos, n_init, sot_idx, finished;
+  int32_t last, penult;
+  int32_t last_ts, pad;
+};
+
 struct DecodeParams {
   int B, V, D, H, L, n_ctx;
   int eot, no_speech, no_timestamps, timestamp_begin;
@@ -53,6 +59,7 @@
   int trace;
   int head_single;
   int split_ln;
+  int head_loader;
   int packed;
   int keep_layers;
   int keep_vocab;
@@ -117,6 +124,7 @@
   int32_t* n_gen = nullptr;
   int32_t* finished = nullptr;
   int32_t* last_ts = nullptr;
+  HeadState* head_state = nullptr;
   int32_t* out_n = nullptr;
   float* sum_logprob = nullptr;
   int32_t* n_logprob = nullptr;
diff --git a/mlx-swift-audio_amd/csrc/whisper_decode.hip b/mlx-swift-audio_amd/csrc/whisper_decode.hip
--- a/mlx-swift-audio_amd/csrc/whisper_decode.hip
+++ b/mlx-swift-audio_amd/csrc/whisper_decode.hip
@@ -155,7 +155,7 @@
   p.eot = o->eot; p.no_speech = o->no_speech; p.no_timestamps = o->no_timestamps; p.timestamp_begin = o->timestamp_begin;
   p.timestamps = o->timestamps ? 1 : 0; p.max_tokens = o->max_tokens;
   p.max_initial_ts = o->max_initial_timestamp_index; p.max_new_tokens = o->max_new_tokens;
-  p.trace = w->trace ? 1 : 0; p.head_single = (w->debug_flags & 2) ? 1 : 0; p.split_ln = (w->debug_flags & 4) ? 1 : 0;
+  p.trace = w->trace ? 1 : 0; p.head_single = (w->debug_flags & 2) ? 1 : 0; p.split_ln = (w->debug_flags & 4) ? 1 : 0; p.head_loader = (w->debug_flags & 32) ? 1 : 0;
   p.packed = w->use_packed ? w->q_bits : 0;
   const bool resident = dec_cache_policy(w, p);
   if (w->trace)
@@ -237,7 +237,10 @@
     w->graph_valid = true;
   }
 
-  if (dec_head_is_split(p)) dec_launch_embed_ln(w, w->dec[0].attn_ln, s);
+  if (dec_head_is_split(p)) {
+    dec_launch_embed_ln(w, w->dec[0].attn_ln, s);
+    dec_launch_head_state_init(w, s);
+  }
   int prof_rec = mia_prof_begin(ctx, MIA_PROF_DECODE, 0.0);
   const int prof_kept = resident ? mia_prof_begin(ctx, MIA_PROF_DECODE_KEPT, 0.0) : -1;
   int steps_run = 0;
@@ -447,7 +450,7 @@
 
 extern "C" int mia_whisper_set_debug(mia_whisper* w, int flags) {
   if (!w) return MIA_ERR_MODEL_NOT_LOADED;
-  MIA_CHECK_ARG(w->ctx, flags >= 0 && (flags & ~23) == 0, "set_debug: flags must be a combination of 1, 2, 4 and 16 (got %d)", flags);
+  MIA_CHECK_ARG(w->ctx, flags >= 0 && (flags & ~55) == 0, "set_debug: flags must be a combination of 1, 2, 4, 16 and 32 (got %d)", flags);
   w->debug_flags = flags;
   return MIA_OK;
 }
diff --git a/mlx-swift-audio_amd/csrc/whisper_encode.hip b/mlx-swift-audio_amd/csrc/whisper_encode.hip
--- a/mlx-swift-audio_amd/csrc/whisper_encode.hip
+++ b/mlx-swift-audio_amd/csrc/whisper_encode.hip
@@ -73,6 +73,7 @@
   A(n_gen, (size_t)B * 4, true);
   A(finished, (size_t)B * 4, true);
   A(last_ts, (size_t)B * 4, true);
+  A(head_state, (size_t)B * sizeof(HeadState), true);
   A(out_n, (size_t)B * 4, true);
   A(sum_logprob, (size_t)B * 4, true);
   A(n_logprob, (size_t)B * 4, true);
@@ -101,7 +102,7 @@
   w->mel_pad = n.mel_pad; w->conv1_out = n.conv1_out; w->x = n.x; w->h = n.h; w->qk = n.qk; w->vt = n.vt; w->att = n.att; w->g = n.g;
   w->feat = n.feat; w->enc_part = n.enc_part; w->enc_stat = n.enc_stat; w->cross_k = n.cross_k; w->cross_v = n.cross_v; w->self_k = n.self_k; w->self_v = n.self_v; w->dx = n.dx; w->dh = n.dh;
   w->dq = n.dq; w->da = n.da; w->dg = n.dg; w->partial = n.partial; w->dstat = n.dstat; w->logits = n.logits; w->tokens = n.tokens; w->n_gen = n.n_gen;
-  w->finished = n.finished; w->last_ts = n.last_ts; w->out_n = n.out_n; w->sum_logprob = n.sum_logprob; w->n_logprob = n.n_logprob;
+  w->finished = n.finished; w->last_ts = n.last_ts; w->head_state = n.head_state; w->out_n = n.out_n; w->sum_logprob = n.sum_logprob; w->n_logprob = n.n_logprob;
   w->no_speech = n.no_speech; w->uniforms = n.uniforms; w->out_tokens = n.out_tokens; w->out_avg = n.out_avg; w->clip = n.clip;
   for (void* q : w->batch_allocs) (void)hipFree(q);
   w->batch_allocs.swap(fresh);
diff --git a/mlx-swift-audio_amd/ops.py b/mlx-swift-audio_amd/ops.py
--- a/mlx-swift-audio_amd/ops.py
+++ b/mlx-swift-audio_amd/ops.py
@@ -273,8 +273,7 @@
     return wf, st
 
 
-def skinny_gemm(ctx: _lib.Context, **d) -> None:
-    lib = ctx.lib
+def _skinny_desc(d: dict) -> SkinnyDesc:
     unknown = set(d) - {n for n, _ in SkinnyDesc._fields_}
     assert not unknown, f"not a mia_skinny_desc field: {sorted(unknown)}"
     desc = SkinnyDesc()
@@ -289,4 +288,14 @@
             desc.ldo = _ld(d.get("out"), v)
         else:
             setattr(desc, name, {"S": 1, "rs_scale": 1.0}.get(name, 0) if v is None else v)
-    _run(ctx, lambda: lib.mia_op_skinny_gemm(ctx.h, C.byref(desc)))
+    return desc
+
+
+def skinny_gemm(ctx: _lib.Context, **d) -> None:
+    desc = _skinny_desc(d)
+    _run(ctx, lambda: ctx.lib.mia_op_skinny_gemm(ctx.h, C.byref(desc)))
+
+
+def skinny_gemm_variant(ctx: _lib.Context, variant: int, **d) -> None:
+    desc = _skinny_desc(d)
+    _run(ctx, lambda: ctx.lib.mia_op_skinny_gemm_variant(ctx.h, C.byref(desc), int(variant)))
```

After: 4911 audio-sec/s (median of 2 runs). No clear change (+0.1%).
